# RemoteSensingTools/vSmartMOM.jl

Measured on AMD Instinct MI355X. Metric: spectral-points/s (whole node) for rt_run, O2-A band, higher is better.
Workload: dtype f64

## Files before the change

include/vsmartmom_hip.h:

```cpp
#ifndef VSMARTMOM_HIP_H
#define VSMARTMOM_HIP_H

#include <stddef.h>
#include <stdint.h>

#ifdef __cplusplus
extern "C" {
#endif

typedef enum vsm_status {
  VSM_OK = 0,
  VSM_ERR_INVALID_ARG = 1,
  VSM_ERR_UNSUPPORTED = 2,
  VSM_ERR_HIP = 3,
  VSM_ERR_NO_DEVICE = 4
} vsm_status;

typedef enum vsm_iface {
  VSM_IFACE_00 = 0,
  VSM_IFACE_01 = 1,
  VSM_IFACE_10 = 2,
  VSM_IFACE_11 = 3
} vsm_iface;

// ... 172 lines not shown
int vsm_elemental_lin_mix_f64(const vsm_quad_f64* q, int S, int m, int ndoubl, const double* dtau, const double* varpi,
                              const double* tau_sum, const double* F0, int ncomp, int ncomp_total, const double* Zc_pp,
                              const double* Zc_mp, int zsel, const double* fz, int p_layer, const double* dtau_dot,
                              const double* varpi_dot, const double* tau_sum_dot, const double* zdcoef,
                              const vsm_added_f64* added, const vsm_added_lin_f64* added_lin, void* stream);
int vsm_elemental_lin_mix_f32(const vsm_quad_f32* q, int S, int m, int ndoubl, const float* dtau, const float* varpi,
                              const float* tau_sum, const float* F0, int ncomp, int ncomp_total, const float* Zc_pp,
                              const float* Zc_mp, int zsel, const float* fz, int p_layer, const float* dtau_dot,
                              const float* varpi_dot, const float* tau_sum_dot, const float* zdcoef,
                              const vsm_added_f32* added, const vsm_added_lin_f32* added_lin, void* stream);
size_t vsm_doubling_lin_work_elems(int N, int S, int P);
int vsm_doubling_lin_f64(int N, int n_stokes, int S, int ndoubl, double* expk, const double* dtau_dot_all, double mu0,
                         int n_active, const vsm_added_f64* added, const vsm_added_lin_f64* added_lin, double* work,
                         void* stream);
int vsm_doubling_lin_f32(int N, int n_stokes, int S, int ndoubl, float* expk, const float* dtau_dot_all, float mu0,
                         int n_active, const vsm_added_f32* added, const vsm_added_lin_f32* added_lin, float* work,
                         void* stream);
size_t vsm_interaction_lin_work_elems(int N, int S, int P);
int vsm_interaction_lin_f64(int iface, int N, int S, const vsm_composite_f64* comp, const vsm_composite_lin_f64* comp_lin,
                            const vsm_added_f64* added, const vsm_added_lin_f64* added_lin, double* work, void* stream);
int vsm_interaction_lin_f32(int iface, int N, int S, const vsm_composite_f32* comp, const vsm_composite_lin_f32* comp_lin,
                            const vsm_added_f32* added, const vsm_added_lin_f32* added_lin, float* work, void* stream);
int vsm_interaction_lin_range_f64(int iface, int N, int S, const vsm_composite_f64* comp, const vsm_composite_lin_f64* comp_lin,
                                  const vsm_added_f64* added, const vsm_added_lin_f64* added_lin, int p_lo, int p_hi, double* work,
                                  void* stream);
int vsm_interaction_lin_range_f32(int iface, int N, int S, const vsm_composite_f32* comp, const vsm_composite_lin_f32* comp_lin,
                                  const vsm_added_f32* added, const vsm_added_lin_f32* added_lin, int p_lo, int p_hi, float* work,
                                  void* stream);
int vsm_copy_added_to_composite_lin_f64(int N, int S, const vsm_added_lin_f64* added_lin,
                                        const vsm_composite_lin_f64* comp_lin, void* stream);
int vsm_copy_added_to_composite_lin_f32(int N, int S, const vsm_added_lin_f32* added_lin,
                                        const vsm_composite_lin_f32* comp_lin, void* stream);
int vsm_lambertian_surface_lin_f64(const vsm_quad_f64* q, int S, int m, double albedo, int iparam, const double* tau_sum,
                                   const double* tau_sum_dot, int p_layer, const double* F0, const vsm_added_f64* added,
                                   const vsm_added_lin_f64* added_lin, void* stream);
int vsm_lambertian_surface_lin_f32(const vsm_quad_f32* q, int S, int m, float albedo, int iparam, const float* tau_sum,
                                   const float* tau_sum_dot, int p_layer, const float* F0, const vsm_added_f32* added,
                                   const vsm_added_lin_f32* added_lin, void* stream);
int vsm_postprocess_vza_lin_f64(int N, int n_stokes, int S, int nV, int P, const int* row0_h, const double* w_h,
                                const double* Jdot0_m, const double* Jdot0_p, double* Rdot, double* Tdot, void* stream);
int vsm_postprocess_vza_lin_f32(int N, int n_stokes, int S, int nV, int P, const int* row0_h, const float* w_h,
                                const float* Jdot0_m, const float* Jdot0_p, float* Rdot, float* Tdot, void* stream);

int vsm_lambertian_surface_spectral_f64(const vsm_quad_f64* q, int S, int m, const double* albedo, const double* tau_sum,
                                        const vsm_added_f64* added, void* stream);
int vsm_lambertian_surface_spectral_f32(const vsm_quad_f32* q, int S, int m, const float* albedo, const float* tau_sum,
                                        const vsm_added_f32* added, void* stream);

typedef struct vsm_coxmunk_f64 {
  double wind_speed, n_water_re, n_water_im, whitecap_albedo;
  int include_whitecaps, shadowing;
} vsm_coxmunk_f64;
typedef struct vsm_coxmunk_f32 {
  float wind_speed, n_water_re, n_water_im, whitecap_albedo;
  int include_whitecaps, shadowing;
} vsm_coxmunk_f32;
int vsm_coxmunk_reflectance_f64(const vsm_coxmunk_f64* surf, const vsm_quad_f64* q, int m, int nphi, const double* phi,
                                const double* wphi, double* rho, double* drho_dU, void* stream);
int vsm_coxmunk_reflectance_f32(const vsm_coxmunk_f32* surf, const vsm_quad_f32* q, int m, int nphi, const float* phi,
                                const float* wphi, float* rho, float* drho_dU, void* stream);
int vsm_brdf_surface_f64(const vsm_quad_f64* q, int S, int m, const double* rho, const double* tau_sum,
                         const vsm_added_f64* added, void* stream);
int vsm_brdf_surface_f32(const vsm_quad_f32* q, int S, int m, const float* rho, const float* tau_sum,
                         const vsm_added_f32* added, void* stream);
int vsm_brdf_surface_lin_f64(const vsm_quad_f64* q, int S, int m, const double* rho, const double* drho, int iparam,
                             const double* tau_sum, const double* tau_sum_dot, int p_layer, const double* F0,
                             const vsm_added_f64* added, const vsm_added_lin_f64* added_lin, void* stream);
int vsm_brdf_surface_lin_f32(const vsm_quad_f32* q, int S, int m, const float* rho, const float* drho, int iparam,
                             const float* tau_sum, const float* tau_sum_dot, int p_layer, const float* F0,
                             const vsm_added_f32* added, const vsm_added_lin_f32* added_lin, void* stream);
int vsm_interaction_hdrf_f64(const vsm_quad_f64* q, int S, int m, const vsm_composite_f64* comp,
                             const vsm_added_f64* added_surface, double* hdr_J, double* bhr_uw, double* bhr_dw, void* stream);
int vsm_interaction_hdrf_f32(const vsm_quad_f32* q, int S, int m, const vsm_composite_f32* comp,
                             const vsm_added_f32* added_surface, float* hdr_J, float* bhr_uw, float* bhr_dw, void* stream);
int vsm_postprocess_vza_hdrf_f64(int N, int n_stokes, int S, int nV, const int* row0_h, const double* w_h, const double* hdr_J,
                                 double* hdr, void* stream);
int vsm_postprocess_vza_hdrf_f32(int N, int n_stokes, int S, int nV, const int* row0_h, const float* w_h, const float* hdr_J,
                                 float* hdr, void* stream);
int vsm_coxmunk_ss_correction_f64(const vsm_coxmunk_f64* surf, int n_stokes, int S, int nV, const double* mu_v_h,
                                  const double* dphi_h, double mu0, int m_max, int nphi, const double* phi,
                                  const double* wphi, const double* tau_total, double* coef, double* R_SFI, void* stream);
int vsm_coxmunk_ss_correction_f32(const vsm_coxmunk_f32* surf, int n_stokes, int S, int nV, const float* mu_v_h,
                                  const float* dphi_h, float mu0, int m_max, int nphi, const float* phi, const float* wphi,
                                  const float* tau_total, float* coef, float* R_SFI, void* stream);

int vsm_compute_Z_moments_f64(const vsm_quad_f64* q, int m, int lmax, const double* greek, double* Zpp, double* Zmp,
                              void* stream);
int vsm_compute_Z_moments_f32(const vsm_quad_f32* q, int m, int lmax, const double* greek, float* Zpp, float* Zmp,
                              void* stream);
int vsm_layer_optics_f64(int S, int L, int nAer, const double* tau_rayl, const double* tau_abs, double varpi_cabannes,
                         const double* tau_aer, const double* ssa, const double* ftrunc, const int* mode, double* tau,
                         double* varpi, double* tau_sum, double* fcomp, double* max_tau_varpi, void* stream);
int vsm_layer_optics_f32(int S, int L, int nAer, const double* tau_rayl, const double* tau_abs, double varpi_cabannes,
                         const double* tau_aer, const double* ssa, const double* ftrunc, const int* mode, float* tau,
                         float* varpi, float* tau_sum, float* fcomp, float* max_tau_varpi, void* stream);
int vsm_layer_dtau_f64(int S, int L, const int* ndoubl, const double* tau, double* dtau, void* stream);
int vsm_layer_dtau_f32(int S, int L, const int* ndoubl, const float* tau, float* dtau, void* stream);
int vsm_layer_optics_lin_f64(int S_full, int lo, int S, int L, int nAer, int nGas, int P, const double* tau_rayl,
                             const double* tau_abs, double varpi_cabannes, const double* tau_aer, const double* ssa,
                             const double* ftrunc, const double* tau_abs_dot, const double* tau_aer_dot,
                             const double* ssa_dot, const double* ftrunc_dot, const int* ndoubl, double* dtau_dot_all,
                             double* varpi_dot, double* tau_sum_dot, double* fz, double* zdcoef, void* stream);
int vsm_layer_optics_lin_f32(int S_full, int lo, int S, int L, int nAer, int nGas, int P, const double* tau_rayl,
                             const double* tau_abs, double varpi_cabannes, const double* tau_aer, const double* ssa,
                             const double* ftrunc, const double* tau_abs_dot, const double* tau_aer_dot,
                             const double* ssa_dot, const double* ftrunc_dot, const int* ndoubl, float* dtau_dot_all,
                             float* varpi_dot, float* tau_sum_dot, float* fz, float* zdcoef, void* stream);
int vsm_layer_expk_f64(int S, const double* dtau, double mu0, double* expk, void* stream);
int vsm_layer_expk_f32(int S, const float* dtau, float mu0, float* expk, void* stream);

int vsm_layer_forward_f64(const vsm_quad_f64* q, int S, int m, int ndoubl, const double* dtau, const double* varpi,
                          const double* tau_sum, const double* F0, const double* Zpp, const double* Zmp, long long z_stride,
                          int toa, const vsm_composite_f64* comp, const vsm_added_f64* added_scratch, void* stream);
int vsm_layer_forward_f32(const vsm_quad_f32* q, int S, int m, int ndoubl, const float* dtau, const float* varpi,
                          const float* tau_sum, const float* F0, const float* Zpp, const float* Zmp, long long z_stride,
                          int toa, const vsm_composite_f32* comp, const vsm_added_f32* added_scratch, void* stream);

int vsm_layer_forward_multi_f64(const vsm_quad_f64* q, int S, int nm, const int* m, int ndoubl, const double* dtau,
                                const double* varpi, const double* tau_sum, const double* F0, int ncomp,
                                const double* const* Zpp, const double* const* Zmp, long long z_stride, const double* fcomp,
                                double* z_scratch, int toa, const vsm_composite_f64* comps, const vsm_added_f64* added_scratch,
                                void* stream);
int vsm_layer_forward_multi_f32(const vsm_quad_f32* q, int S, int nm, const int* m, int ndoubl, const float* dtau,
                                const float* varpi, const float* tau_sum, const float* F0, int ncomp, const float* const* Zpp,
                                const float* const* Zmp, long long z_stride, const float* fcomp, float* z_scratch, int toa,
                                const vsm_composite_f32* comps, const vsm_added_f32* added_scratch, void* stream);

int vsm_layer_thermal_fused(int N, int is_f64);
int vsm_layer_forward_thermal_f64(const vsm_quad_f64* q, int S, int ndoubl, const double* dtau, const double* varpi,
                                  const double* thermal_B, int ncomp, const double* Zpp, const double* Zmp, long long z_stride,
                                  const double* fcomp, int toa, const vsm_composite_f64* comp, void* stream);
int vsm_layer_forward_thermal_f32(const vsm_quad_f32* q, int S, int ndoubl, const float* dtau, const float* varpi,
                                  const float* thermal_B, int ncomp, const float* Zpp, const float* Zmp, long long z_stride,
                                  const float* fcomp, int toa, const vsm_composite_f32* comp, void* stream);

int vsm_layer_forward_mix_f64(const vsm_quad_f64* q, int S, int m, int ndoubl, const double* dtau, const double* varpi,
                              const double* tau_sum, const double* F0, int ncomp, const double* Zpp_comp,
                              const double* Zmp_comp, const double* fcomp, double* z_scratch, int toa,
                              const vsm_composite_f64* comp, const vsm_added_f64* added_scratch, void* stream);
int vsm_layer_forward_mix_f32(const vsm_quad_f32* q, int S, int m, int ndoubl, const float* dtau, const float* varpi,
                              const float* tau_sum, const float* F0, int ncomp, const float* Zpp_comp, const float* Zmp_comp,
                              const float* fcomp, float* z_scratch, int toa, const vsm_composite_f32* comp,
                              const vsm_added_f32* added_scratch, void* stream);
int vsm_mix_Z_f64(int N, int S, int ncomp, const double* Zpp_comp, const double* Zmp_comp, const double* fcomp, double* Zpp,
                  double* Zmp, void* stream);
int vsm_mix_Z_f32(int N, int S, int ncomp, const float* Zpp_comp, const float* Zmp_comp, const float* fcomp, float* Zpp,
                  float* Zmp, void* stream);
int vsm_mix_Z_moments_f64(int N, int S, int ncomp, int nm, const double* const* Zpp_comp_h, const double* const* Zmp_comp_h, int single,
                          const double* fcomp, double* Zpp, double* Zmp, void* stream);
int vsm_mix_Z_moments_f32(int N, int S, int ncomp, int nm, const float* const* Zpp_comp_h, const float* const* Zmp_comp_h, int single,
                          const float* fcomp, float* Zpp, float* Zmp, void* stream);

typedef struct vsm_run vsm_run;
enum { VSM_RUN_SOURCES_ONLY = 1 };
int vsm_run_supported(int N, int n_stokes, int coupling);
size_t vsm_run_workspace_bytes(int N, int n_stokes, int S, int nm, const int* coupling_h);
int vsm_run_supported_f32(int N, int n_stokes, int coupling);
size_t vsm_run_workspace_bytes_f32(int N, int n_stokes, int S, int nm, const int* coupling_h);
int vsm_run_create_f64(const vsm_quad_f64* q, int S, int nm, const int* m_h, const int* coupling_h, void* workspace,
                       size_t workspace_bytes, vsm_run** run);
int vsm_run_create_f32(const vsm_quad_f32* q, int S, int nm, const int* m_h, const int* coupling_h, void* workspace,
                       size_t workspace_bytes, vsm_run** run);
int vsm_run_create_ex_f64(const vsm_quad_f64* q, int S, int nm, const int* m_h, const int* coupling_h, void* workspace,
                          size_t workspace_bytes, unsigned flags, vsm_run** run);
int vsm_run_create_ex_f32(const vsm_quad_f32* q, int S, int nm, const int* m_h, const int* coupling_h, void* workspace,
                          size_t workspace_bytes, unsigned flags, vsm_run** run);
int vsm_run_layer_f64(vsm_run* run, int ndoubl, const double* dtau, const double* varpi, const double* tau_sum,
                      const double* F0, int ncomp, const double* const* Zpp, const double* const* Zmp, long long z_stride,
                      const double* fcomp, int toa, const int* layer_coupling_h, void* stream);
int vsm_run_layer_f32(vsm_run* run, int ndoubl, const float* dtau, const float* varpi, const float* tau_sum,
                      const float* F0, int ncomp, const float* const* Zpp, const float* const* Zmp, long long z_stride,
                      const float* fcomp, int toa, const int* layer_coupling_h, void* stream);
int vsm_run_export_f64(vsm_run* run, const vsm_composite_f64* comps, void* stream);
int vsm_run_export_f32(vsm_run* run, const vsm_composite_f32* comps, void* stream);
int vsm_run_import_f64(vsm_run* run, const vsm_composite_f64* comps, void* stream);
int vsm_run_import_f32(vsm_run* run, const vsm_composite_f32* comps, void* stream);
int vsm_run_destroy(vsm_run* run);
int vsm_stokes_coupling_f64(int N, int n_stokes, int nblocks, const double* Zpp, const double* Zmp, int* mask_d, void* stream);
int vsm_stokes_coupling_f32(int N, int n_stokes, int nblocks, const float* Zpp, const float* Zmp, int* mask_d, void* stream);

typedef struct vsm_added_rs_f64 {
  double *ier_mp, *iet_pp, *ier_pm, *iet_mm;
  double *ieJ0_p, *ieJ0_m;
  int K;
  int reserved;
} vsm_added_rs_f64;
typedef struct vsm_added_rs_f32 {
  float *ier_mp, *iet_pp, *ier_pm, *iet_mm;
  float *ieJ0_p, *ieJ0_m;
  int K;
  int reserved;
} vsm_added_rs_f32;
typedef struct vsm_composite_rs_f64 {
  double *ieR_mp, *ieR_pm, *ieT_pp, *ieT_mm;
  double *ieJ0_p, *ieJ0_m;
  int K;
  int reserved;
} vsm_composite_rs_f64;
typedef struct vsm_composite_rs_f32 {
  float *ieR_mp, *ieR_pm, *ieT_pp, *ieT_mm;
  float *ieJ0_p, *ieJ0_m;
  int K;
  int reserved;
} vsm_composite_rs_f32;
typedef struct vsm_rrs_f64 {
  const int* shift;
  const double* varpi_ie;
  const double* fscatt;
  const double* Zpp;
  const double* Zmp;
} vsm_rrs_f64;
typedef struct vsm_rrs_f32 {
  const int* shift;
  const float* varpi_ie;
  const float* fscatt;
  const float* Zpp;
  const float* Zmp;
} vsm_rrs_f32;
int vsm_elemental_inelastic_rrs_f64(const vsm_quad_f64* q, int S, int m, int ndoubl, const double* dtau,
                                    const double* tau_sum, const double* F0, const vsm_rrs_f64* rs,
                                    const vsm_added_rs_f64* added_rs, void* stream);
int vsm_elemental_inelastic_rrs_f32(const vsm_quad_f32* q, int S, int m, int ndoubl, const float* dtau,
                                    const float* tau_sum, const float* F0, const vsm_rrs_f32* rs,
                                    const vsm_added_rs_f32* added_rs, void* stream);
size_t vsm_doubling_inelastic_work_elems(int N, int S, int K);
int vsm_doubling_inelastic_rrs_f64(int N, int n_stokes, int S, int ndoubl, double* expk, const int* shift,
                                   const vsm_added_f64* added, const vsm_added_rs_f64* added_rs, double* work, void* stream);
int vsm_doubling_inelastic_rrs_f32(int N, int n_stokes, int S, int ndoubl, float* expk, const int* shift,
                                   const vsm_added_f32* added, const vsm_added_rs_f32* added_rs, float* work, void* stream);
size_t vsm_interaction_inelastic_work_elems(int N, int S, int K);
int vsm_interaction_inelastic_rrs_f64(int iface, int N, int S, const int* shift, const vsm_composite_f64* comp,
                                      const vsm_composite_rs_f64* comp_rs, const vsm_added_f64* added,
                                      const vsm_added_rs_f64* added_rs, double* work, void* stream);
int vsm_interaction_inelastic_rrs_f32(int iface, int N, int S, const int* shift, const vsm_composite_f32* comp,
                                      const vsm_composite_rs_f32* comp_rs, const vsm_added_f32* added,
                                      const vsm_added_rs_f32* added_rs, float* work, void* stream);
int vsm_copy_added_to_composite_ie_f64(int N, int S, const vsm_added_rs_f64* added_rs, const vsm_composite_rs_f64* comp_rs,
                                       void* stream);
int vsm_copy_added_to_composite_ie_f32(int N, int S, const vsm_added_rs_f32* added_rs, const vsm_composite_rs_f32* comp_rs,
                                       void* stream);
int vsm_postprocess_vza_ie_f64(int N, int n_stokes, int S, int K, int nV, const int* row0_h, const double* w_h,
                               const double* ieJ0_m, const double* ieJ0_p, double* ieR, double* ieT, void* stream);
int vsm_postprocess_vza_ie_f32(int N, int n_stokes, int S, int K, int nV, const int* row0_h, const float* w_h,
                               const float* ieJ0_m, const float* ieJ0_p, float* ieR, float* ieT, void* stream);

size_t vsm_level_radiance_work_elems(int N, int S);
int vsm_level_radiance_f64(int N, int n_stokes, int S, int nV, const int* row0_h, const double* w_h, const double* top_R_pm,
                           const double* top_J0_p, const double* bot_R_mp, long long bot_stride, const double* bot_J0_m,
                           double* uw, double* dw, double* dw_full, double* uw_full, double* work, void* stream);
int vsm_level_radiance_f32(int N, int n_stokes, int S, int nV, const int* row0_h, const float* w_h, const float* top_R_pm,
                           const float* top_J0_p, const float* bot_R_mp, long long bot_stride, const float* bot_J0_m,
                           float* uw, float* dw, float* dw_full, float* uw_full, float* work, void* stream);
int vsm_level_radiance_oplevel_f64(int N, int n_stokes, int S, int nV, const int* row0_h, const double* w_h,
                                   const double* top_R_pm, const double* top_J0_p, const double* bot_R_mp, long long bot_stride,
                                   const double* bot_J0_m, double* uw, double* dw, double* dw_full, double* uw_full,
                                   double* work, void* stream);
int vsm_level_radiance_oplevel_f32(int N, int n_stokes, int S, int nV, const int* row0_h, const float* w_h,
                                   const float* top_R_pm, const float* top_J0_p, const float* bot_R_mp, long long bot_stride,
                                   const float* bot_J0_m, float* uw, float* dw, float* dw_full, float* uw_full, float* work,
                                   void* stream);

int vsm_test_lds_mm_f64(int N, int S, const double* A, const double* B, double* C, void* stream);
int vsm_test_lds_mm_f32(int N, int S, const float* A, const float* B, float* C, void* stream);
int vsm_test_lds_inv_f64(int N, int S, const double* A, double* X, int mode, int* path_out, void* stream);
int vsm_test_lds_inv_f32(int N, int S, const float* A, float* X, int mode, int* path_out, void* stream);

int vsm_test_poison_lds(void* stream);

#ifdef __cplusplus
}
#endif
#endif
```

vsmartmom.jl_amd/_lib.py:

```python
from __future__ import annotations

import ctypes as C
import os

_HERE = os.path.dirname(os.path.abspath(__file__))
LIB_PATH = os.environ.get("VSM_LIB_PATH") or os.path.join(_HERE, "lib", "libvsmartmom_hip.so")


class VSMError(RuntimeError):
    pass


class vsm_quad_f64(C.Structure):
    _fields_ = [("mu", C.c_void_p), ("wt", C.c_void_p), ("N", C.c_int), ("n_stokes", C.c_int),
                ("i_mu0", C.c_int), ("mu0", C.c_double)]


class vsm_quad_f32(C.Structure):
    _fields_ = [("mu", C.c_void_p), ("wt", C.c_void_p), ("N", C.c_int), ("n_stokes", C.c_int),
                ("i_mu0", C.c_int), ("mu0", C.c_float)]


class vsm_added(C.Structure):
    _fields_ = [("r_mp", C.c_void_p), ("t_pp", C.c_void_p), ("r_pm", C.c_void_p), ("t_mm", C.c_void_p),
                ("j0_p", C.c_void_p), ("j0_m", C.c_void_p), ("mat_stride", C.c_longlong),
                ("d_symmetric", C.c_int), ("reserved", C.c_int)]


class vsm_composite(C.Structure):
    _fields_ = [("R_mp", C.c_void_p), ("R_pm", C.c_void_p), ("T_pp", C.c_void_p), ("T_mm", C.c_void_p),
                ("J0_p", C.c_void_p), ("J0_m", C.c_void_p)]


class vsm_added_lin(C.Structure):
    _fields_ = [("ap_r_mp", C.c_void_p), ("ap_t_pp", C.c_void_p), ("ap_r_pm", C.c_void_p), ("ap_t_mm", C.c_void_p),
                ("ap_J0_p", C.c_void_p), ("ap_J0_m", C.c_void_p), ("P", C.c_int), ("reserved", C.c_int),
                ("mat_stride", C.c_longlong)]


class vsm_composite_lin(C.Structure):
    _fields_ = [("R_mp", C.c_void_p), ("R_pm", C.c_void_p), ("T_pp", C.c_void_p), ("T_mm", C.c_void_p),
                ("J0_p", C.c_void_p), ("J0_m", C.c_void_p), ("P", C.c_int), ("reserved", C.c_int)]


class vsm_added_rs(C.Structure):
    _fields_ = [("ier_mp", C.c_void_p), ("iet_pp", C.c_void_p), ("ier_pm", C.c_void_p), ("iet_mm", C.c_void_p),
                ("ieJ0_p", C.c_void_p), ("ieJ0_m", C.c_void_p), ("K", C.c_int), ("reserved", C.c_int)]


class vsm_composite_rs(C.Structure):
    _fields_ = [("ieR_mp", C.c_void_p), ("ieR_pm", C.c_void_p), ("ieT_pp", C.c_void_p), ("ieT_mm", C.c_void_p),
                ("ieJ0_p", C.c_void_p), ("ieJ0_m", C.c_void_p), ("K", C.c_int), ("reserved", C.c_int)]


class vsm_coxmunk_f64(C.Structure):
    _fields_ = [("wind_speed", C.c_double), ("n_water_re", C.c_double), ("n_water_im", C.c_double),
                ("whitecap_albedo", C.c_double), ("include_whitecaps", C.c_int), ("shadowing", C.c_int)]


class vsm_coxmunk_f32(C.Structure):
    _fields_ = [("wind_speed", C.c_float), ("n_water_re", C.c_float), ("n_water_im", C.c_float),
                ("whitecap_albedo", C.c_float), ("include_whitecaps", C.c_int), ("shadowing", C.c_int)]


class vsm_rrs(C.Structure):
    _fields_ = [("shift", C.c_void_p), ("varpi_ie", C.c_void_p), ("fscatt", C.c_void_p), ("Zpp", C.c_void_p),
                ("Zmp", C.c_void_p)]


_P, _I, _LL, _SZ = C.c_void_p, C.c_int, C.c_longlong, C.c_size_t

_SIGS = {
    "vsm_version": (_I, []),
    "vsm_last_error": (C.c_char_p, []),
    "vsm_build_id": (C.c_char_p, []),
    "vsm_device_count": (_I, [C.POINTER(_I)]),
    "vsm_device_name": (_I, [_I, C.c_char_p, _SZ]),
    "vsm_sync": (_I, [_P]),
    "vsm_release_scratch": (_I, []),
    "vsm_device_status": (_I, [C.POINTER(_I), _I, _P]),
    "vsm_fused_max_n": (_I, [_I]),
    "vsm_layer_thermal_fused": (_I, [_I, _I]),
    "vsm_doubling_work_elems": (_SZ, [_I, _I]),
    "vsm_interaction_work_elems": (_SZ, [_I, _I]),
    "vsm_batched_mul_{T}": (_I, [_I, _I, _I, _I, _P, _LL, _P, _LL, _P, _P]),
    "vsm_batch_inv_{T}": (_I, [_I, _I, _P, _P, _P, _P]),
    "vsm_batch_solve_{T}": (_I, [_I, _I, _I, _P, _P, _P, _P, _P, _P]),
    "vsm_elemental_doubling_{T}": (_I, [_P, _I, _I, _I, _P, _P, _P, _P, _P, _P, _LL, _P, _P]),
    "vsm_layer_forward_{T}": (_I, [_P, _I, _I, _I, _P, _P, _P, _P, _P, _P, _LL, _I, _P, _P, _P]),
    "vsm_layer_forward_multi_{T}": (_I, [_P, _I, _I, _P, _I, _P, _P, _P, _P, _I, _P, _P, _LL, _P, _P, _I, _P, _P, _P]),
    "vsm_layer_forward_thermal_{T}": (_I, [_P, _I, _I, _P, _P, _P, _I, _P, _P, _LL, _P, _I, _P, _P]),
    "vsm_layer_forward_mix_{T}": (_I, [_P, _I, _I, _I, _P, _P, _P, _P, _I, _P, _P, _P, _P, _I, _P, _P, _P]),
    "vsm_mix_Z_{T}": (_I, [_I, _I, _I, _P, _P, _P, _P, _P, _P]),
    "vsm_mix_Z_moments_{T}": (_I, [_I, _I, _I, _I, _P, _P, _I, _P, _P, _P, _P]),
    "vsm_elemental_{T}": (_I, [_P, _I, _I, _I, _P, _P, _P, _P, _P, _P, _LL, _P, _P]),
    "vsm_doubling_{T}": (_I, [_I, _I, _I, _I, _P, _P, _P, _P]),
    "vsm_noscat_layer_{T}": (_I, [_P, _I, _P, _P, _P]),
    "vsm_thermal_source_{T}": (_I, [_P, _I, _P, _P, _P, _P, _P]),
    "vsm_copy_added_to_composite_{T}": (_I, [_I, _I, _P, _P, _P]),
    "vsm_interaction_{T}": (_I, [_I, _I, _I, _P, _P, _P, _P]),
    "vsm_interaction_oplevel_{T}": (_I, [_I, _I, _I, _P, _P, _P, _P]),
    "vsm_lambertian_surface_{T}": (_I, [_P, _I, _I, "{R}", _P, _P, _P]),
    "vsm_postprocess_vza_{T}": (_I, [_I, _I, _I, _I, _P, _P, _P, _P, _P, _P, _P]),
    "vsm_compute_Z_moments_{T}": (_I, [_P, _I, _I, _P, _P, _P, _P]),
    "vsm_layer_optics_{T}": (_I, [_I, _I, _I, _P, _P, C.c_double, _P, _P, _P, _P, _P, _P, _P, _P, _P, _P]),
    "vsm_layer_dtau_{T}": (_I, [_I, _I, _P, _P, _P, _P]),
    "vsm_layer_optics_lin_{T}": (_I, [_I, _I, _I, _I, _I, _I, _I, _P, _P, C.c_double, _P, _P, _P, _P, _P, _P, _P, _P, _P, _P, _P,
                                      _P, _P, _P]),
    "vsm_layer_expk_{T}": (_I, [_I, _P, "{R}", _P, _P]),
    "vsm_coxmunk_reflectance_{T}": (_I, [_P, _P, _I, _I, _P, _P, _P, _P, _P]),
    "vsm_lambertian_surface_spectral_{T}": (_I, [_P, _I, _I, _P, _P, _P, _P]),
    "vsm_brdf_surface_{T}": (_I, [_P, _I, _I, _P, _P, _P, _P]),
    "vsm_brdf_surface_lin_{T}": (_I, [_P, _I, _I, _P, _P, _I, _P, _P, _I, _P, _P, _P, _P]),
    "vsm_interaction_hdrf_{T}": (_I, [_P, _I, _I, _P, _P, _P, _P, _P, _P]),
    "vsm_postprocess_vza_hdrf_{T}": (_I, [_I, _I, _I, _I, _P, _P, _P, _P, _P]),
    "vsm_coxmunk_ss_correction_{T}": (_I, [_P, _I, _I, _I, _P, _P, "{R}", _I, _I, _P, _P, _P, _P, _P, _P]),
    "vsm_doubling_lin_work_elems": (_SZ, [_I, _I, _I]),
    "vsm_interaction_lin_work_elems": (_SZ, [_I, _I, _I]),
    "vsm_elemental_lin_{T}": (_I, [_P, _I, _I, _I, _P, _P, _P, _P, _P, _P, _LL, _I, _P, _P, _P, _P, _P, _LL, _LL, _P, _P, _P]),
    "vsm_elemental_lin_fold_{T}": (_I, [_P, _I, _I, _I, _I, _P, _P, _P, _P, _P, _P, _LL, _I, _P, _P, _P, _P, _P, _P]),
    "vsm_elemental_lin_mix_{T}": (_I, [_P, _I, _I, _I, _P, _P, _P, _P, _I, _I, _P, _P, _I, _P, _I, _P, _P, _P, _P, _P, _P, _P]),
    "vsm_doubling_lin_{T}": (_I, [_I, _I, _I, _I, _P, _P, "{R}", _I, _P, _P, _P, _P]),
    "vsm_interaction_lin_{T}": (_I, [_I, _I, _I, _P, _P, _P, _P, _P, _P]),
    "vsm_interaction_lin_range_{T}": (_I, [_I, _I, _I, _P, _P, _P, _P, _I, _I, _P, _P]),
    "vsm_copy_added_to_composite_lin_{T}": (_I, [_I, _I, _P, _P, _P]),
    "vsm_lambertian_surface_lin_{T}": (_I, [_P, _I, _I, "{R}", _I, _P, _P, _I, _P, _P, _P, _P]),
    "vsm_postprocess_vza_lin_{T}": (_I, [_I, _I, _I, _I, _I, _P, _P, _P, _P, _P, _P, _P]),
    "vsm_doubling_inelastic_work_elems": (_SZ, [_I, _I, _I]),
    "vsm_interaction_inelastic_work_elems": (_SZ, [_I, _I, _I]),
    "vsm_elemental_inelastic_rrs_{T}": (_I, [_P, _I, _I, _I, _P, _P, _P, _P, _P, _P]),
    "vsm_doubling_inelastic_rrs_{T}": (_I, [_I, _I, _I, _I, _P, _P, _P, _P, _P, _P]),
    "vsm_interaction_inelastic_rrs_{T}": (_I, [_I, _I, _I, _P, _P, _P, _P, _P, _P, _P]),
    "vsm_copy_added_to_composite_ie_{T}": (_I, [_I, _I, _P, _P, _P]),
    "vsm_postprocess_vza_ie_{T}": (_I, [_I, _I, _I, _I, _I, _P, _P, _P, _P, _P, _P, _P]),
    "vsm_run_supported": (_I, [_I, _I, _I]),
    "vsm_run_workspace_bytes": (_SZ, [_I, _I, _I, _I, _P]),
    "vsm_run_supported_f32": (_I, [_I, _I, _I]),
    "vsm_run_workspace_bytes_f32": (_SZ, [_I, _I, _I, _I, _P]),
    "vsm_run_create_{T}": (_I, [_P, _I, _I, _P, _P, _P, _SZ, _P]),
    "vsm_run_create_ex_{T}": (_I, [_P, _I, _I, _P, _P, _P, _SZ, C.c_uint, _P]),
    "vsm_run_layer_{T}": (_I, [_P, _I, _P, _P, _P, _P, _I, _P, _P, _LL, _P, _I, _P, _P]),
    "vsm_run_export_{T}": (_I, [_P, _P, _P]),
    "vsm_run_import_{T}": (_I, [_P, _P, _P]),
    "vsm_run_destroy": (_I, [_P]),
    "vsm_stokes_coupling_{T}": (_I, [_I, _I, _I, _P, _P, _P, _P]),
    "vsm_level_radiance_work_elems": (_SZ, [_I, _I]),
    "vsm_level_radiance_{T}": (_I, [_I, _I, _I, _I, _P, _P, _P, _P, _P, _LL, _P, _P, _P, _P, _P, _P, _P]),
    "vsm_level_radiance_oplevel_{T}": (_I, [_I, _I, _I, _I, _P, _P, _P, _P, _P, _LL, _P, _P, _P, _P, _P, _P, _P]),
    "vsm_test_lds_mm_{T}": (_I, [_I, _I, _P, _P, _P, _P]),
    "vsm_test_lds_inv_{T}": (_I, [_I, _I, _P, _P, _I, _P, _P]),
    "vsm_test_poison_lds": (_I, [_P]),
}


def exported_symbols():
    out = []
    for name in _SIGS:
        if "{T}" in name:
            out += [name.format(T="f64"), name.format(T="f32")]
        else:
            out.append(name)
    return out


_lib = None


def lib():
    global _lib
    if _lib is not None:
        return _lib
    if not os.path.exists(LIB_PATH):
        raise VSMError("libvsmartmom_hip.so not found at %s -- run `python -c 'import __graft_entry__ as g; g.build()'` "
                       "(there is no CPU fallback)" % LIB_PATH)
    L = C.CDLL(LIB_PATH)
    for name, (res, args) in _SIGS.items():
        for T, R in (("f64", C.c_double), ("f32", C.c_float)):
            n = name.format(T=T)
            try:
                fn = getattr(L, n)
            except AttributeError:
                if os.environ.get("VSM_LIB_PATH"):
                    if "{T}" not in name:
                        break
                    continue
                raise
            fn.restype = res
            fn.argtypes = [R if a == "{R}" else a for a in args]
            if "{T}" not in name:
                break
    _lib = L
    return L


def build_info() -> dict:
    import json
    info = {"source_hash": lib().vsm_build_id().decode() if hasattr(lib(), "vsm_build_id") else None}
    try:
        with open(os.path.join(os.path.dirname(LIB_PATH), "BUILD_INFO.json")) as f:
            side = json.load(f)
        if side.get("source_hash") == info["source_hash"]:
            info.update(side)
    except (OSError, ValueError):
        pass
    return info


def poison(t):
    if os.environ.get("VSM_POISON_WORK"):
        t.fill_(float("nan"))
    return t


def check(rc):
    if rc != 0:
        raise VSMError("libvsmartmom_hip: status %d: %s" % (rc, lib().vsm_last_error().decode()))


last_device_status = [0, 0, 0, 0]


def check_device_status(what="rt_run"):
    global last_device_status
    flags = (C.c_int * 4)()
    check(lib().vsm_device_status(flags, 1, None))
    last_device_status = list(flags)
    if flags[0] & 1:
        raise VSMError("%s: singular matrix in an in-kernel inverse ((I - R r) or (I - r r) has an exactly zero pivot)" % what)
    if flags[0] & 2:
        raise VSMError("%s: NaN / Inf operand in an in-kernel inverse" % what)
    if flags[0] & 4:
        raise VSMError("%s: a phase matrix handed to vsm_run_layer has a non-zero element outside the declared Stokes coupling "
                       "(VSM_DEVSTAT_MASK): the native run dropped that coupling" % what)


def suffix(dtype) -> str:
    import torch
    if dtype == torch.float64:
        return "f64"
    if dtype == torch.float32:
        return "f32"
    raise VSMError("unsupported float type %r (Float64 / Float32 only)" % (dtype,))


def call(name, dtype, *args):
    fn = getattr(lib(), "%s_%s" % (name, suffix(dtype)))
    check(fn(*args))
```

vsmartmom.jl_amd/core_rt.py:

```python
from __future__ import annotations

import ctypes as C
import dataclasses
import math
import os
from dataclasses import dataclass
from typing import List, Optional

import numpy as np
import torch

from . import _lib
from . import host_model as H
from .architectures import GPU, CPU, architecture, array_type, devi, synchronize_if_gpu, to_host

IFACE = {"00": 0, "01": 1, "10": 2, "11": 3}
MOMENT_BATCH = 4
MOMENT_BATCH_MAX = 24
MOMENT_BATCHING = True
THERMAL_FUSION = True
NATIVE_RUN = True
NATIVE_SOURCES_ONLY = True
NATIVE_DROPIN = True
REFERENCE_ORDER = False


def _require_gpu(arch):
    if not isinstance(arch, GPU):
        raise _lib.VSMError("vsmartmom.jl_amd provides the MI355X path only; architecture %r has no compute path here "
                            "(no CPU fallback by design)" % (arch,))
    if not torch.cuda.is_available():
        raise _lib.VSMError("no MI355X visible to HIP (torch.cuda.is_available() is False)")
    if arch.device_index != torch.cuda.current_device():
        raise _lib.VSMError("architecture GPU(%d) is not the current HIP device (%d): one process per GPU -- call "
                            "torch.cuda.set_device(%d) first" % (arch.device_index, torch.cuda.current_device(),
                                                                 arch.device_index))


def _torch_dtype(FT):
    return torch.float64 if np.dtype(FT) == np.float64 else torch.float32


def _stream_ptr():
    return C.c_void_p(torch.cuda.current_stream().cuda_stream)


def _ptr(t: Optional[torch.Tensor]):
    return C.c_void_p(0 if t is None else t.data_ptr())


def to_device_matrix(A: np.ndarray, arch, FT) -> torch.Tensor:
    A = np.asarray(A, dtype=FT)
    if A.ndim == 2:
        A = A[None]
    return array_type(arch)(np.ascontiguousarray(A.transpose(0, 2, 1)))


def from_device_matrix(t: torch.Tensor) -> np.ndarray:
    return to_host(t).transpose(0, 2, 1).copy()


def batched_mul(A: torch.Tensor, B: torch.Tensor) -> torch.Tensor:
    _require_gpu(architecture(A))
    vec = B.dim() == 2
    S, K, M = A.shape
    Nc = 1 if vec else B.shape[1]
    kb = B.shape[1] if vec else B.shape[2]
    if kb != K or B.shape[0] not in (S, 1):
        raise _lib.VSMError("batched_mul: dimension mismatch %s x %s" % (tuple(A.shape), tuple(B.shape)))
    A, B = A.contiguous(), B.contiguous()
    Cout = torch.empty((S, M) if vec else (S, Nc, M), dtype=A.dtype, device=A.device)
    sb = 0 if B.shape[0] == 1 and S > 1 else K * Nc
    _lib.call("vsm_batched_mul", A.dtype, M, Nc, K, S, _ptr(A), M * K, _ptr(B), sb, _ptr(Cout), _stream_ptr())
    return Cout


def batch_inv_(X: torch.Tensor, A: torch.Tensor, info: Optional[torch.Tensor] = None):
    _require_gpu(architecture(A))
    S, N, N2 = A.shape
    if N != N2 or X.shape != A.shape:
        raise _lib.VSMError("batch_inv!: square batches of equal shape required")
    _lib.call("vsm_batch_inv", A.dtype, N, S, _ptr(A), _ptr(X), _ptr(info), _stream_ptr())
    return X


def batch_solve_(X: torch.Tensor, A: torch.Tensor, B: torch.Tensor, info: Optional[torch.Tensor] = None):
    _require_gpu(architecture(A))
    S, N, N2 = A.shape
    nrhs = 1 if B.dim() == 2 else B.shape[1]
    if N != N2 or B.shape[0] != S or B.shape[-1] != N or X.shape != B.shape:
        raise _lib.VSMError("batch_solve!: A [N,N,S] and B, X [N,Nrhs,S] required")
    work = _lib.poison(torch.empty_like(A))
    _lib.call("vsm_batch_solve", A.dtype, N, nrhs, S, _ptr(A.contiguous()), _ptr(B.contiguous()), _ptr(X), _ptr(work), _ptr(info),
              _stream_ptr())
    return X


def batched_pointer_cache(A):
    return None


@dataclass
class DeviceQuad:
    host: H.QuadPoints
    mu: torch.Tensor
    wt: torch.Tensor
    n_stokes: int
    dtype: torch.dtype

    def cstruct(self):
        cls = _lib.vsm_quad_f64 if self.dtype == torch.float64 else _lib.vsm_quad_f32
        return cls(self.mu.data_ptr(), self.wt.data_ptr(), int(self.mu.numel()), self.n_stokes, self.host.imu0,
                   self.host.mu0)


def device_quad(qp: H.QuadPoints, pol: H.PolarizationType, arch, FT) -> DeviceQuad:
    conv = array_type(arch)
    return DeviceQuad(qp, conv(qp.qp_muN.astype(FT)), conv(qp.wt_muN.astype(FT)), pol.n, _torch_dtype(FT))


class AddedLayer:

    def __init__(self, FT, arch, N, nSpec, shared=False, d_symmetric=0):
        dev, dt = devi(arch), _torch_dtype(FT)
        sm = 1 if shared else nSpec
        z = lambda: torch.zeros((sm, N, N), dtype=dt, device=dev)
        self.r_mp, self.t_pp = z(), z()
        self.d_symmetric = int(d_symmetric)
        self.r_pm, self.t_mm = (None, None) if self.d_symmetric else (z(), z())
        self.j0_p = torch.zeros((nSpec, N), dtype=dt, device=dev)
        self.j0_m = torch.zeros((nSpec, N), dtype=dt, device=dev)
        self.N, self.nSpec, self.shared, self.dtype = N, nSpec, shared, dt

    def cstruct(self):
        return _lib.vsm_added(self.r_mp.data_ptr(), self.t_pp.data_ptr(),
                              0 if self.r_pm is None else self.r_pm.data_ptr(),
                              0 if self.t_mm is None else self.t_mm.data_ptr(),
                              self.j0_p.data_ptr(), self.j0_m.data_ptr(), 0 if self.shared else self.N * self.N,
                              self.d_symmetric, 0)


def _composite_field(name):
    def fget(self):
        return self.materialize()._arr[name]

    def fset(self, value):
        self.materialize()._arr[name] = value
    return property(fget, fset)


class CompositeLayer:

    def __init__(self, FT, arch, N, nSpec):
        dev, dt = devi(arch), _torch_dtype(FT)
        z = lambda: torch.zeros((nSpec, N, N), dtype=dt, device=dev)
        self._native = None
        self._sources_only = False
        self._native_ws = None
        self._arr = dict(R_mp=z(), R_pm=z(), T_pp=z(), T_mm=z(), J0_p=torch.zeros((nSpec, N), dtype=dt, device=dev),
                         J0_m=torch.zeros((nSpec, N), dtype=dt, device=dev))
        self.N, self.nSpec, self.dtype = N, nSpec, dt

    R_mp, R_pm, T_pp = _composite_field("R_mp"), _composite_field("R_pm"), _composite_field("T_pp")
    T_mm, J0_p, J0_m = _composite_field("T_mm"), _composite_field("J0_p"), _composite_field("J0_m")

    def materialize(self):
        slot = self._native
        if slot is None:
            return self
        self._native = None
        try:
            cc = (_lib.vsm_composite * 1)(self._cstruct_raw())
            _lib.call("vsm_run_export", self.dtype, slot.run, cc, _stream_ptr())
        finally:
            _lib.lib().vsm_run_destroy(slot.run)
# ... 578 lines not shown
                key = (type(model.surface).__name__, dataclasses.astuple(model.surface), m)
                cache = self.__dict__.setdefault("_rho_cache", {})
                if key not in cache:
                    if len(cache) > 4 * (model.m_max + 1):
                        cache.clear()
                    cache[key] = reflectance(model.surface, self.dq, m, self.arch, FT)[0]
                rho = cache[key]
            self.moments.append(dict(m=m, layers=layers, iface_surface=tags[-1], rho=rho, tau_sum_surface=self.tau_sum[L, lo:hi]))
        all11 = all(t == "11" for t in tags)
        fused_ok = self.N <= _lib.lib().vsm_fused_max_n(8 if np.dtype(FT) == np.float64 else 4)
        dsym = self.pol.n if (all11 and fused_ok and not self.full_added_layer) else 0
        if self.added is None or self.added.d_symmetric != dsym:
            self.added = make_added_layer(FT, self.arch, (self.N, self.N), self.S, d_symmetric=dsym)

    def _prepare_host(self):
        model, FT, L, S_full = self.model, self.FT, self.Nz, self.S_full
        conv = array_type(self.arch)
        nds = tags = maxima = None
        for m in range(model.m_max + 1):
            Zc_pp, Zc_mp, lods = H.constructLayerOpticsComponents(model, m)
            self.Zc[m][0].copy_(to_device_matrix(Zc_pp, self.arch, FT))
            self.Zc[m][1].copy_(to_device_matrix(Zc_mp, self.arch, FT))
            if m > 0:
                continue
            tags, tau_sum_all = H.extractEffectiveProps(lods, FT)
            nds, maxima = [], []
            zcomp = []
            for iz, lo in enumerate(lods):
                tau_full = np.atleast_1d(lo.tau).astype(FT)
                varpi_full = np.broadcast_to(np.asarray(lo.varpi, dtype=FT), tau_full.shape)
                tw = float(np.max(tau_full * varpi_full))
                scatter = tw > 2 * np.finfo(FT).eps
                dtau_full, nd = (H.get_dtau_ndoubl(tau_full, varpi_full, self.qp, FT, model.numerics) if scatter else (tau_full, 0))
                nds.append(nd)
                maxima.append(tw)
                self.tau[iz].copy_(conv(tau_full))
                self.varpi[iz].copy_(conv(np.ascontiguousarray(varpi_full)))
                self.dtau[iz].copy_(conv(np.ascontiguousarray(dtau_full)))
                self.tau_sum[iz].copy_(conv(tau_sum_all[:, iz].astype(FT)))
                if lo.coef.ndim == 1:
                    zcomp.append((False, int(np.argmax(lo.coef))))
                else:
                    zcomp.append((True, 0))
                    self.fcomp[iz].copy_(conv(np.ascontiguousarray(lo.coef.astype(FT))))
            self.tau_sum[L].copy_(conv(tau_sum_all[:, -1].astype(FT)))
            self.zcomp = zcomp
        self._compute_coupling()
        self._assemble(nds, tags, maxima)

    def _compute_coupling(self):
        C_ = int(self.Zc[0][0].shape[0])
        if not self.host_optics and getattr(self, "coupling_comp", None) is not None:
            return
        if getattr(self, "_coupling_d", None) is None:
            self._coupling_d = torch.zeros((len(self.Zc), C_), dtype=torch.int32, device=self.dev)
        for m, (Zpp, Zmp) in enumerate(self.Zc):
            _lib.call("vsm_stokes_coupling", self.dt, self.N, self.pol.n, C_, _ptr(Zpp), _ptr(Zmp),
                      C.c_void_p(self._coupling_d[m].data_ptr()), _stream_ptr())
        self.coupling_comp = self._coupling_d.cpu().numpy().astype(np.int64)
        self.coupling = [int(np.bitwise_or.reduce(row)) for row in self.coupling_comp]

    def _layer_coupling(self, m, iz):
        mixed, k = self.zcomp[iz]
        row = self.coupling_comp[m]
        return int(np.bitwise_or.reduce(row)) if mixed else int(row[k])

    def run(self, trace: Optional[list] = None, streams: Optional[list] = None):
        model, pol, FT = self.model, self.pol, self.FT
        self.R_SFI.zero_()
        self.T_SFI.zero_()
        self.hdr.zero_()
        if self.S == 0:
            return self.R_SFI, self.T_SFI
        self.added.j0_p.zero_()
        eps2 = 2 * np.finfo(FT).eps
        has_noscat = any(ly["props"].max_tau_varpi <= eps2 for ly in self.moments[0]["layers"])
        sequential = trace is not None or not MOMENT_BATCHING or has_noscat or REFERENCE_ORDER
        want = max(MOMENT_BATCH, min(MOMENT_BATCH_MAX, 4096 // max(self.S, 1)))
        nb = 1 if sequential else min(want, len(self.moments))
        while len(self._composites) < nb:
            self._composites.append(make_composite_layer(FT, self.arch, (self.N, self.N), self.S))
        native = self._native_moments() if trace is None and not has_noscat and not REFERENCE_ORDER else set()
        walk_src = streams is None and trace is None and not has_noscat
        for c in self._composites:
            c._sources_only = walk_src and REFERENCE_ORDER
        for g0 in range(0, len(self.moments), nb):
            group = self.moments[g0:g0 + nb]
            comps = self._composites[:len(group)]
            nat = [k for k in range(len(group)) if (g0 + k) in native]
            if nat:
                self._run_layers_native([group[k] for k in nat], [comps[k] for k in nat], sources_only=streams is None)
            rest = [k for k in range(len(group)) if (g0 + k) not in native]
            group_l, comps_l = [group[k] for k in rest], [comps[k] for k in rest]
            for iz in range(self.Nz if rest else 0):
                ly0 = group_l[0]["layers"][iz]
                if len(group_l) > 1 and ly0["props"].max_tau_varpi > eps2 and (iz == 0 or ly0["iface"] == "11"):
                    layer_forward_multi_(ly0["tau_sum"], ly0["dtau"], self.F0, [mom["layers"][iz]["props"] for mom in group_l],
                                         [mom["m"] for mom in group_l], ly0["nd"], self.dq, iz == 0, comps_l, self.added)
                    continue
                for mom, comp in zip(group_l, comps_l):
                    ly = mom["layers"][iz]
                    rt_kernel_(pol, self.added, comp, ly["props"], ly["iface"], ly["tau_sum"], mom["m"], self.dq,
                               self.arch, iz + 1, self.F0, FT, model.numerics, dtau=ly["dtau"], ndoubl=ly["nd"], trace=trace,
                               work=self.work, keep_added=has_noscat)
            for mom, comp in zip(group, comps):
                m = mom["m"]
                weight = FT(0.5 / math.pi) if m == 0 else FT(1.0 / math.pi)
                create_surface_layer_(model.surface, self.added_surface, m, self.dq, mom["tau_sum_surface"], rho=mom["rho"])
                interaction_(mom["iface_surface"], comp, self.added_surface, work=self.work)
                if self.compute_hdrf:
                    interaction_hdrf_(pol, comp, self.added_surface, m, self.dq, model.vza, model.vaz, self.qp, float(weight),
                                      self.hdr_J, self.hdr, self.bhr_uw, self.bhr_dw)
                postprocessing_vza_(pol, comp, model.vza, model.vaz, self.qp, m, float(weight), self.R_SFI, self.T_SFI)
                thermal_pass = self.thermal_B is not None and (m == 0 or (m == 1 and self._thermal_carry))
                if thermal_pass:
                    self._thermal_slot(mom, float(weight))
                if streams is not None:
                    Jm, Jp = comp.J0_m.clone(), comp.J0_p.clone()
                    if thermal_pass:
                        Jm += self._th_comp.J0_m
                        Jp += self._th_comp.J0_p
                    streams.append(dict(m=m, weight=float(weight), R_mp=comp.R_mp.clone(), T_pp=comp.T_pp.clone(), J0_m=Jm, J0_p=Jp))
        for c in self._composites:
            c._sources_only = False
        if isinstance(model.surface, H.CoxMunkSurface) and self.ss_correction:
            apply_ss_correction_(self.R_SFI, model.surface, pol, model.vza, model.vaz, self.qp.mu0,
                                 self.moments[-1]["tau_sum_surface"], model.m_max, self.arch, FT)
        return self.R_SFI, self.T_SFI

    def _native_moments(self):
        if not NATIVE_RUN or getattr(self, "coupling", None) is None or not self.moments:
            return set()
        eps2 = 2 * np.finfo(self.FT).eps
        for iz, ly in enumerate(self.moments[0]["layers"]):
            p = ly["props"]
            if p.max_tau_varpi <= eps2 or (iz > 0 and ly["iface"] != "11") or (p.fcomp is not None and p.fcomp.shape[1] > 4):
                return set()
        return {i for i, mom in enumerate(self.moments) if run_supported(self.dt, self.N, self.pol.n, int(self.coupling[mom["m"]]))}

    def _run_layers_native(self, group, comps, sources_only: bool = True, export_at=None):
        L = _lib.lib()
        nm, N, S, ns = len(group), self.N, self.S, self.pol.n
        marr = (C.c_int * nm)(*[int(mom["m"]) for mom in group])
        carr = (C.c_int * nm)(*[int(self.coupling[mom["m"]]) for mom in group])
        nbytes = run_workspace_bytes(self.dt, N, ns, S, nm, carr)
        ws = getattr(self, "_native_ws", None)
        if ws is None or ws.numel() * 8 < nbytes:
            ws = self._native_ws = _lib.poison(torch.empty(max(nbytes // 8, 2), dtype=torch.float64, device=self.dev))
        q = self.dq.cstruct()
        run = C.c_void_p()
        flags = 1 if (sources_only and NATIVE_SOURCES_ONLY) else 0
        _lib.call("vsm_run_create_ex", self.dt, C.byref(q), S, nm, marr, carr, _ptr(ws), nbytes, flags, C.byref(run))
        try:
            for iz in range(self.Nz):
                ly0 = group[0]["layers"][iz]
                props = [mom["layers"][iz]["props"] for mom in group]
                p0 = props[0]
                zpp = (C.c_void_p * nm)(*[p.Zpp.data_ptr() for p in props])
                zmp = (C.c_void_p * nm)(*[p.Zmp.data_ptr() for p in props])
                ncomp = 0 if p0.fcomp is None else int(p0.fcomp.shape[1])
                lc = (C.c_int * nm)(*[self._layer_coupling(mom["m"], iz) for mom in group])
                run_layer_native_(run, nm, int(ly0["nd"]), ly0["dtau"], p0.varpi, ly0["tau_sum"], self.F0, ncomp, zpp, zmp,
                                  0 if ncomp else p0.z_stride, p0.fcomp, iz == 0, lc, self.dt)
                if export_at and (iz + 1) in export_at:
                    cc = (type(comps[0].cstruct()) * nm)(*[c.cstruct() for c in comps])
                    _lib.call("vsm_run_export", self.dt, run, cc, _stream_ptr())
                    export_at[iz + 1](comps)
            cc = (type(comps[0].cstruct()) * nm)(*[c.cstruct() for c in comps])
            _lib.call("vsm_run_export", self.dt, run, cc, _stream_ptr())
        finally:
            L.vsm_run_destroy(run)

    def _thermal_slot(self, mom, weight):
        model, pol, FT = self.model, self.pol, self.FT
        N, S = self.N, self.S
        m = mom["m"]
        if getattr(self, "_th_added", None) is None:
            self._th_added = make_added_layer(FT, self.arch, (N, N), S, d_symmetric=0)
            self._th_surf = make_added_layer(FT, self.arch, (N, N), S, shared=not self.spectral_surface)
            self._th_comp = make_composite_layer(FT, self.arch, (N, N), S)
            self._th_F0 = torch.zeros_like(self.F0)
            self._th_ones = torch.ones(max(S, 1), dtype=self.dt, device=self.dev)
        added, comp = self._th_added, self._th_comp
        q = self.dq.cstruct()
        eps2 = 2 * np.finfo(FT).eps
        scat = [ly["props"].max_tau_varpi > eps2 for ly in mom["layers"]]
        keep_state = not self.thermal_reset_noscat
        if m == 0:
            added.j0_p.zero_()
            added.j0_m.zero_()
            self._thermal_carry = keep_state and any(scat) and not scat[0] and model.m_max >= 1
        fused = (THERMAL_FUSION and m == 0 and (all(scat) or not keep_state)
                 and _lib.lib().vsm_layer_thermal_fused(N, 1 if FT == np.float64 else 0) != 0)
        for iz, ly in enumerate(mom["layers"]):
            props = ly["props"]
            scatter = scat[iz]
            if (fused and scatter and (iz == 0 or ly["iface"] == "11") and iz < self.thermal_B.shape[0]
                    and (props.fcomp is None or props.fcomp.shape[1] <= 4)):
                c = comp.cstruct()
                ncomp = 0 if props.fcomp is None else int(props.fcomp.shape[1])
                _lib.call("vsm_layer_forward_thermal", self.dt, C.byref(q), S, ly["nd"], _ptr(ly["dtau"]), _ptr(props.varpi),
                          _ptr(self.thermal_B[iz]), ncomp, _ptr(props.Zpp), _ptr(props.Zmp),
                          0 if ncomp else props.z_stride, _ptr(props.fcomp), 1 if iz == 0 else 0, C.byref(c), _stream_ptr())
                continue
            if scatter:
                elemental_(pol, ly["tau_sum"], ly["dtau"], self._th_F0, props.materialize(), m, ly["nd"], self.dq, added)
                if m == 0 and iz < self.thermal_B.shape[0]:
                    a = added.cstruct()
                    _lib.call("vsm_thermal_source", self.dt, C.byref(q), S, _ptr(ly["dtau"]), _ptr(props.varpi),
                              _ptr(self.thermal_B[iz]), C.byref(a), _stream_ptr())
                self._th_ones.fill_(1.0)
                doubling_(pol, self._th_ones, ly["nd"], added)
            elif keep_state:
                jm = added.j0_m.clone()
                zero_added_noscat_(added, props.tau, self.dq)
                added.j0_m.copy_(jm)
            else:
                zero_added_noscat_(added, props.tau, self.dq)
                added.j0_p.zero_()
                added.j0_m.zero_()
            if iz == 0:
                copy_added_to_composite_(comp, added)
            else:
                interaction_(ly["iface"], comp, added, oplevel=True, work=self.work)
        create_surface_layer_(model.surface, self._th_surf, m, self.dq, mom["tau_sum_surface"], rho=mom["rho"])
        self._th_surf.j0_p.zero_()
        self._th_surf.j0_m.zero_()
        interaction_(mom["iface_surface"], comp, self._th_surf, oplevel=True, work=self.work)
        postprocessing_vza_(pol, comp, model.vza, model.vaz, self.qp, m, weight, self.R_SFI, self.T_SFI)

    def run_graph(self):
        if getattr(self, "_graph", None) is None:
            if self.added.d_symmetric == 0 or any(ly["props"].fcomp is not None for ly in self.moments[0]["layers"]):
                raise _lib.VSMError("run_graph(): only scenes that run entirely in the fused layer kernels (every layer "
                                    "scattering, N within the on-chip limit, one scatterer per layer) can be captured")
            gs = torch.cuda.Stream()
            gs.wait_stream(torch.cuda.current_stream())
            with torch.cuda.stream(gs):
                self.run()
            torch.cuda.synchronize()
            g = torch.cuda.CUDAGraph()
            with torch.cuda.graph(g, stream=gs):
                self.run()
            self._graph, self._graph_stream = g, gs
        self._graph.replay()
        return self.R_SFI, self.T_SFI

    def results_host(self):
        return to_host(self.R_SFI).transpose(2, 1, 0).copy(), to_host(self.T_SFI).transpose(2, 1, 0).copy()

    def results_host_full(self):
        R, T = self.results_host()
        return (R, T, np.zeros_like(R), np.zeros_like(T), to_host(self.hdr).transpose(2, 1, 0).copy(),
                to_host(self.bhr_uw)[:, 0].copy(), to_host(self.bhr_dw)[:, 0].copy())

    def flops_per_point(self) -> float:
        N = float(self.N)
        tot = 0.0
        for mom in self.moments:
            for iz, ly in enumerate(mom["layers"]):
                tot += ly["nd"] * (12 * N ** 3 + 8 * N ** 2)
                if iz > 0:
                    tot += 24 * N ** 3 + 8 * N ** 2
            tot += 24 * N ** 3 + 8 * N ** 2
        return tot


def prepare_scene(model: H.RTModel, spec_slice: Optional[slice] = None) -> Scene:
    return Scene(model, spec_slice)


@dataclass
class StreamRTResult:
    qp_mu: np.ndarray
    i_mu0: int
    mu0: float
    pol_n: int
    weight: List[float]
    R_mp_per_m: List[np.ndarray]
    T_pp_per_m: List[np.ndarray]
    J_m_per_m: List[np.ndarray]
    J_p_per_m: List[np.ndarray]
    tau_total: np.ndarray
    tau_rayl: np.ndarray
    tau_abs: np.ndarray


def rt_run_streams(model: H.RTModel) -> StreamRTResult:
    scene = prepare_scene(model)
    scene.compute_hdrf = False
    st: list = []
    scene.run(streams=st)
    synchronize_if_gpu()
    st.sort(key=lambda d: d["m"])
    mat = lambda t: from_device_matrix(t).transpose(1, 2, 0).copy()
    vec = lambda t: to_host(t).T[:, None, :].copy()
    qp = model.quad_points
    FT = model.float_type
    return StreamRTResult(np.asarray(qp.qp_mu, dtype=FT).copy(), int(qp.imu0) + 1, float(qp.mu0), model.polarization_type.n,
                          [d["weight"] for d in st], [mat(d["R_mp"]) for d in st], [mat(d["T_pp"]) for d in st],
                          [vec(d["J0_m"]) for d in st], [vec(d["J0_p"]) for d in st],
                          (np.asarray(model.tau_rayl) + np.asarray(model.tau_abs)).astype(FT), np.asarray(model.tau_rayl, dtype=FT),
                          np.asarray(model.tau_abs, dtype=FT))


def rt_run(model: H.RTModel, trace: Optional[list] = None, full_output: bool = False):
# ... 7 lines not shown
```

vsmartmom.jl_amd/csrc/vsm_native.hip:

```cpp
#include <stdlib.h>

#include <vector>

#include "vsm_native_dev.h"
#include "vsm_native_run.h"

#ifndef VSM_NATIVE_PARK_RT
#define VSM_NATIVE_PARK_RT 3
#endif

namespace vsm {

struct nlayer_comps {
  double* c[NSUB_MAX];
};

namespace {

template <int RT, int KS>
__device__ __forceinline__ void ned_body(nsmem<RT, (4 * KS + 2 > 16 * RT)>& sm, npos<RT>& p, int n, int gsz, unsigned uvmask, int ndoubl,
                                         const double* __restrict__ img, nstrip<RT>& r_s, nstrip<RT>& t_s, int* status) {
  using G = ngeo<RT>;
  constexpr unsigned dP = 0, dQ = G::AF * 8;
  double* jp = sm.vec[0];
  double* jm = sm.vec[1];
  double* rsg = sm.vec[3];
  const int tid = threadIdx.x;
  constexpr int c1 = 4 * KS, c2 = 4 * KS + 1;
  constexpr bool RID = c2 < G::NP;
  static_assert(RID || KS == 4 * RT, "no spare columns for the source vectors");
  const bool own_wave = RID && p.wave == (c1 >> 4);
  const bool laneA = own_wave && (p.col == c1), laneB = own_wave && (p.col == c2), laneAB = laneA || laneB;
  ncopy_image<RT>(sm.P, img, p);
  ncopy_image<RT>(sm.Q, img + G::AF, p);
  if (tid < G::NP) {
    jp[tid] = img[2 * G::AF + tid];
    jm[tid] = img[2 * G::AF + G::NP + tid];
    const bool uv = (uvmask >> (tid % gsz)) & 1u;
    sm.usg[tid] = uv ? -1.0 : 1.0;
    rsg[tid] = (ndoubl >= 1 && uv) ? -1.0 : 1.0;
  }
  const double expk0 = img[2 * G::AF + 2 * G::NP];
  __builtin_amdgcn_s_waitcnt(0x0F70);
  __syncthreads();
  nload(r_s, dP, p);
  nload(t_s, dQ, p);
  double expk = expk0;
  int slot = 0;
  const ninv_ctx cx{dP, sm.P, sm.gjs, status};
  for (int it = 0; it < ndoubl; ++it) {
    nstrip<RT> W, tt;
    const double fW = laneA ? expk : (laneB ? 1.0 : 0.0), fR = laneB ? expk : 1.0;
    if constexpr (!RID) {
      nmv_rows<RT, KS>(dP, jp, 1.0, sm.mv[0], p);
      nmv_rows<RT, KS>(dP, jm, expk, sm.mv[1], p);
    }
    {
      nstrip<RT> Gs;
      {
        nstrip<RT> E;
        nmm2<RT, KS, true, true>(E, W, dP, r_s, t_s, p);
        if (own_wave) {
#pragma unroll
          for (int ta = 0; ta < RT; ++ta)
#pragma unroll
            for (int r = 0; r < 4; ++r) {
              W.v[ta][r] = fma(r_s.v[ta][r], fW, W.v[ta][r]);
              r_s.v[ta][r] *= fR;
            }
        }
        const double nrm = nnorm(E, n, sm, slot, p);
        if constexpr (!RID) {
          if (tid < G::NP) {
            sm.vec[4][tid] = jm[tid] * expk + sm.mv[0][tid];
            sm.vec[5][tid] = jp[tid] + sm.mv[1][tid];
          }
        }
        ninvert<RT, KS>(ninv_order(nrm, status), E, Gs, n, cx, p);
      }
      nmm<RT, KS, true>(tt, dQ, Gs, p);
    }
    nload(t_s, dQ, p);
    __syncthreads();
    nstore(dP, tt, p);
    __syncthreads();
    if constexpr (!RID) {
      nmv_rows<RT, KS>(dP, sm.vec[4], 1.0, sm.mv[0], p);
      nmv_rows<RT, KS>(dP, sm.vec[5], 1.0, sm.mv[1], p);
    }
    {
      nstrip<RT> tn;
      nmm2<RT, KS, false, true>(r_s, tn, dP, W, t_s, p);
      t_s = tn;
    }
    const double expk_step = expk;
    expk = expk * expk;
    if (own_wave) {
      const double ft = laneB ? expk : 1.0;
#pragma unroll
      for (int ta = 0; ta < RT; ++ta)
#pragma unroll
        for (int r = 0; r < 4; ++r) {
          const double u = ndpp_swap1(r_s.v[ta][r]) * ft;
          t_s.v[ta][r] = laneAB ? u : t_s.v[ta][r];
        }
    }
    if (it + 1 < ndoubl || !RID) __syncthreads();
    if constexpr (!RID) {
      if (tid < G::NP) {
        jm[tid] += sm.mv[0][tid];
        jp[tid] = jp[tid] * expk_step + sm.mv[1][tid];
      }
    }
    if (it + 1 < ndoubl) {
      nstore(dP, r_s, p);
      nstore(dQ, t_s, p);
      __syncthreads();
    }
  }
  if (ndoubl > 0 && own_wave) {
#pragma unroll
    for (int ta = 0; ta < RT; ++ta)
#pragma unroll
      for (int r = 0; r < 4; ++r) {
        const int row = p.row(ta, r);
        double* dpv = laneA ? jp : sm.vec[7];
        double* dmv = laneA ? jm : sm.vec[7];
        dpv[row] = t_s.v[ta][r];
        dmv[row] = r_s.v[ta][r];
        t_s.v[ta][r] = laneAB ? 0.0 : t_s.v[ta][r];
        r_s.v[ta][r] = laneAB ? 0.0 : r_s.v[ta][r];
      }
  }
  __syncthreads();
  if (ndoubl >= 1) {
#pragma unroll
    for (int ta = 0; ta < RT; ++ta)
#pragma unroll
      for (int r = 0; r < 4; ++r) r_s.v[ta][r] *= rsg[p.row(ta, r)];
    if (tid < G::NP) jm[tid] *= rsg[tid];
  }
  __syncthreads();
}

template <int RT, int KS>
__device__ __forceinline__ void nia_body_native(nsmem<RT, (4 * KS + 2 > 16 * RT)>& sm, npos<RT>& p, int n, double* __restrict__ comp, nstrip<RT>& r_s,
                                         nstrip<RT>& t_s, int* status) {
  using G = ngeo<RT>;
  constexpr unsigned dP = 0, dQ = G::AF * 8;
  double* vjp = sm.vec[0];
  double* vjm = sm.vec[1];
  double* vJp = sm.vec[2];
  double* vJm = sm.vec[3];
  double* vs = sm.vec[4];
  double* vz = sm.vec[5];
  const int tid = threadIdx.x;
  double* R_mp = comp + NC_RMP * G::AF;
  double* R_pm = comp + NC_RPM * G::AF;
  double* T_pp = comp + NC_TPP * G::AF;
  double* T_mm = comp + NC_TMM * G::AF;
  double* J0_p = comp + 4 * G::AF;
  double* J0_m = J0_p + G::NP;
  constexpr int c1 = 4 * KS, c2 = 4 * KS + 1;
  constexpr bool RID = c2 < G::NP;
  constexpr bool PARK = VSM_NATIVE_PARK_RT > 0 && (RT == VSM_NATIVE_PARK_RT || RT >= 5);
  const bool own_wave = RID && p.wave == (c1 >> 4);
  const bool laneA = own_wave && (p.col == c1), laneB = own_wave && (p.col == c2);
  int slot = 0;
  const ndpar<RT> dp(sm.usg, p);
  const ninv_ctx cx{dP, sm.P, sm.gjs, status};
  if (tid < G::NP) {
    vJp[tid] = J0_p[tid];
    vJm[tid] = J0_m[tid];
  }
  nstrip<RT> Z, Gs;
  {
    nstrip<RT> A1, A2;
    nld_native(A1, R_pm, p);
    nld_native(A2, T_mm, p);
    nstore(dP, A1, p);
    nstore(dQ, A2, p);
  }
  if (own_wave) {
#pragma unroll
    for (int ta = 0; ta < RT; ++ta)
#pragma unroll
      for (int r = 0; r < 4; ++r) r_s.v[ta][r] = laneB ? vjm[p.row(ta, r)] : r_s.v[ta][r];
  }
  ndsym(t_s, t_s, dp);
  __syncthreads();
  if constexpr (!RID) {
    nmv_rows<RT, KS>(dP, vjm, 1.0, sm.mv[0], p);
    nmv_rows<RT, KS>(dQ, vjm, 1.0, sm.mv[1], p);
  }
  {
    nstrip<RT> E;
    nmm2<RT, KS, true, true>(E, Z, dP, r_s, t_s, p);
    if (own_wave) {
      double* zd = laneB ? vz : sm.vec[7];
#pragma unroll
      for (int ta = 0; ta < RT; ++ta)
#pragma unroll
        for (int r = 0; r < 4; ++r) {
          const int row = p.row(ta, r);
          zd[row] = vJp[row] + E.v[ta][r];
        }
    }
    if constexpr (PARK) nst_native(R_pm, Z, p);
    const double nrm = nnorm(E, n, sm, slot, p);
    if constexpr (!RID) {
      if (tid < G::NP) {
        vz[tid] = vJp[tid] + sm.mv[0][tid];
        vs[tid] = sm.mv[1][tid];
      }
    }
    ninvert<RT, KS>(ninv_order(nrm, status), E, Gs, n, cx, p);
  }
  nstrip<RT> V;
  {
    nstrip<RT> S;
    nmm2<RT, KS, true, true>(S, V, dQ, r_s, t_s, p);
    if (own_wave) {
      double* sd = laneB ? vs : sm.vec[7];
#pragma unroll
      for (int ta = 0; ta < RT; ++ta)
#pragma unroll
        for (int r = 0; r < 4; ++r) sd[p.row(ta, r)] = S.v[ta][r];
    }
    ndsym(r_s, r_s, dp);
    ndsym(t_s, t_s, dp);
    __syncthreads();
    nstore(dQ, S, p);
    nstore(dP, t_s, p);
  }
  __syncthreads();
  {
    nstrip<RT> X, Y;
    nmm<RT, KS, true>(X, dP, Gs, p);
    nmm<RT, KS, true>(Y, dQ, Gs, p);
    __syncthreads();
    nstore(dP, X, p);
    nstore(dQ, Y, p);
  }
  __builtin_amdgcn_sched_barrier(0);
  nstrip<RT> Tpp, Rmp;
  nld_native(Tpp, T_pp, p);
  if constexpr (PARK) nld_native(Z, R_pm, p); else nld_native(Rmp, R_mp, p);
  __syncthreads();
  if constexpr (!RID) {
    nmv_rows<RT, KS>(dP, vz, 1.0, sm.mv[0], p);
    nmv_rows<RT, KS>(dQ, vz, 1.0, sm.mv[1], p);
  }
  if (own_wave) {
#pragma unroll
    for (int ta = 0; ta < RT; ++ta)
#pragma unroll
      for (int r = 0; r < 4; ++r) {
        Tpp.v[ta][r] = laneA ? vz[p.row(ta, r)] : Tpp.v[ta][r];
        if constexpr (!PARK) Rmp.v[ta][r] = laneA ? 0.0 : Rmp.v[ta][r];
      }
  }
  {
    nstrip<RT> acc;
    nmm2<RT, KS, false, true>(r_s, acc, dP, Z, Tpp, p);
    nst_native(R_pm, r_s, p);
    nst_native(T_pp, acc, p);
    if (laneA) {
#pragma unroll
      for (int ta = 0; ta < RT; ++ta)
#pragma unroll
        for (int r = 0; r < 4; ++r) {
          const int row = p.row(ta, r);
          J0_p[row] = vjp[row] + acc.v[ta][r];
        }
    }
  }
  if constexpr (PARK) {
    __builtin_amdgcn_sched_barrier(0);
    nld_native(Rmp, R_mp, p);
    if (own_wave) {
#pragma unroll
      for (int ta = 0; ta < RT; ++ta)
#pragma unroll
        for (int r = 0; r < 4; ++r) Rmp.v[ta][r] = laneA ? 0.0 : Rmp.v[ta][r];
    }
  }
  nmm2<RT, KS>(Rmp, V, dQ, Tpp, Z, p);
  nst_native(R_mp, Rmp, p);
  nst_native(T_mm, V, p);
  if (laneA) {
#pragma unroll
    for (int ta = 0; ta < RT; ++ta)
#pragma unroll
      for (int r = 0; r < 4; ++r) {
        const int row = p.row(ta, r);
        J0_m[row] = vJm[row] + vs[row] + Rmp.v[ta][r];
      }
  }
  if constexpr (!RID) {
    __syncthreads();
    if (tid < G::NP) {
      J0_p[tid] = vjp[tid] + sm.mv[0][tid];
      J0_m[tid] = vJm[tid] + vs[tid] + sm.mv[1][tid];
    }
  }
}

template <int RT, int KS>
__device__ __forceinline__ void nia_body_src(nsmem<RT, (4 * KS + 2 > 16 * RT)>& sm, npos<RT>& p, int n, double* __restrict__ comp,
                                             nstrip<RT>& r_s, nstrip<RT>& t_s, int* status) {
  using G = ngeo<RT>;
  constexpr unsigned dP = 0, dQ = G::AF * 8;
  double* vjp = sm.vec[0];
  double* vjm = sm.vec[1];
  double* vJp = sm.vec[2];
  double* vJm = sm.vec[3];
  double* vu = sm.vec[4];
  double* vtJ = sm.vec[5];
  double* vg = sm.vec[6];
  const int tid = threadIdx.x;
  double* R_pm = comp + NC_RPM * G::AF;
  double* T_mm = comp + NC_TMM * G::AF;
  double* J0_p = comp + 4 * G::AF;
  double* J0_m = J0_p + G::NP;
  constexpr int c1 = 4 * KS, c2 = 4 * KS + 1;
  constexpr bool RID = c2 < G::NP;
  const bool own_wave = RID && p.wave == (c1 >> 4);
  const bool laneA = own_wave && (p.col == c1);
  constexpr bool PARK = VSM_NATIVE_PARK_RT > 0 && (RT == VSM_NATIVE_PARK_RT || RT >= 5);
  int slot = 0;
  const ndpar<RT> dp(sm.usg, p);
  const ninv_ctx cx{dP, sm.P, sm.gjs, status};
  if (tid < G::NP) {
    vJp[tid] = J0_p[tid];
    vJm[tid] = J0_m[tid];
  }
  nstrip<RT> B;
  nld_native(B, R_pm, p);
  nstore(dP, r_s, p);
  nstore(dQ, t_s, p);
  __syncthreads();
  {
    const bool cin = p.col < n;
#pragma unroll
    for (int ta = 0; ta < RT; ++ta)
#pragma unroll
      for (int r = 0; r < 4; ++r) B.v[ta][r] = cin ? B.v[ta][r] : (laneA ? vJp[p.row(ta, r)] : 0.0);
  }
  if constexpr (!RID) {
    nmv_rows<RT, KS>(dP, vJp, 1.0, sm.mv[0], p);
    nmv_rows<RT, KS>(dQ, vJp, 1.0, sm.mv[1], p);
  }
  nstrip<RT> E, Bs;
  double nrm;
  {
    nstrip<RT> Pm;
    nmm2a<RT, KS, true, true>(E, dP, Pm, dQ, B, p);
    ndsym(Bs, t_s, dp);
    ndsym(r_s, r_s, dp);
    if (own_wave) {
#pragma unroll
      for (int ta = 0; ta < RT; ++ta)
#pragma unroll
        for (int r = 0; r < 4; ++r) {
          const int row = p.row(ta, r);
          Bs.v[ta][r] = laneA ? E.v[ta][r] + vjm[row] : Bs.v[ta][r];
          r_s.v[ta][r] = laneA ? Pm.v[ta][r] + vjp[row] : r_s.v[ta][r];
        }
    }
    if constexpr (PARK) nst_native(R_pm, r_s, p);
    nrm = nnorm(E, n, sm, slot, p);
    nstore(dQ, Pm, p);
  }
  if constexpr (!RID) {
    if (tid < G::NP) {
      vu[tid] = sm.mv[0][tid] + vjm[tid];
      vtJ[tid] = sm.mv[1][tid] + vjp[tid];
    }
  }
  nstrip<RT> W;
  {
    nstrip<RT> Gs;
    const int K = ninv_order(nrm, status);
    if (K == 7) ninvert7<RT, KS>(E, Gs, n, cx, p);
    else ninvert<RT, KS>(K, E, Gs, n, cx, p);
    __syncthreads();
    nstore(dP, Gs, p);
  }
  __syncthreads();
  if constexpr (!RID) nmv_rows<RT, KS>(dP, vu, 1.0, vg, p);
  {
    nstrip<RT> Tm;
    nld_native(Tm, T_mm, p);
    if constexpr (PARK) nld_native(r_s, R_pm, p);
    nmm<RT, KS, true>(W, dP, Bs, p);
    __syncthreads();
    nstore(dP, Tm, p);
  }
  __syncthreads();
  if constexpr (!RID) {
    nmv_rows<RT, KS>(dP, vg, 1.0, sm.mv[0], p);
    nmv_rows<RT, KS>(dQ, vg, 1.0, sm.mv[1], p);
  }
  {
    nstrip<RT> Tn;
    nmm2a<RT, KS, true, false>(Tn, dP, r_s, dQ, W, p);
    nst_native(R_pm, r_s, p);
    nst_native(T_mm, Tn, p);
    if (laneA) {
#pragma unroll
      for (int ta = 0; ta < RT; ++ta)
#pragma unroll
        for (int r = 0; r < 4; ++r) {
          const int row = p.row(ta, r);
          J0_p[row] = r_s.v[ta][r];
          J0_m[row] = vJm[row] + Tn.v[ta][r];
        }
    }
  }
  if constexpr (!RID) {
    __syncthreads();
    if (tid < G::NP) {
      J0_m[tid] = vJm[tid] + sm.mv[0][tid];
      J0_p[tid] = vtJ[tid] + sm.mv[1][tid];
    }
  }
}

template <int RT>
struct nio_ref {
  int N;
  double* m[4];
  double* J[2];
  const double* a[4];
  double jpre[2];
  bool al16;
  static constexpr bool REF = true;
  static __device__ __forceinline__ void swap16(double& a, double& b) {
    const unsigned long long ua = __double_as_longlong(a), ub = __double_as_longlong(b);
    const auto lo = __builtin_amdgcn_permlane16_swap((unsigned)ua, (unsigned)ub, false, false);
    const auto hi = __builtin_amdgcn_permlane16_swap((unsigned)(ua >> 32), (unsigned)(ub >> 32), false, false);
    a = __longlong_as_double(((unsigned long long)hi[0] << 32) | lo[0]);
    b = __longlong_as_double(((unsigned long long)hi[1] << 32) | lo[1]);
  }
  typedef double npair16_t __attribute__((ext_vector_type(2)));
  typedef double npair8_t __attribute__((ext_vector_type(2), aligned(8)));
  template <typename PT>
  __device__ __forceinline__ void ldg_even(nstrip<RT>& x, const double* __restrict__ gc, bool cok, int rb) const {
#pragma unroll
    for (int ta = 0; ta < RT; ++ta)
#pragma unroll
      for (int h = 0; h < 2; ++h) {
        const int row = 16 * ta + 8 * h + rb;
        const PT v = *reinterpret_cast<const PT*>(gc + min(row, N - 2));
        const bool ok = cok && row < N;
        double a = ok ? v.x : 0.0, b = ok ? v.y : 0.0;
        swap16(a, b);
        x.v[ta][2 * h] = a;
        x.v[ta][2 * h + 1] = b;
      }
  }
  __device__ __forceinline__ void ldg(nstrip<RT>& x, const double* __restrict__ g, const npos<RT>& p) const {
    const bool cok = p.col < N;
    const int rb = 4 * (p.kq & 1) + 2 * (p.kq >> 1);
    const double* gc = g + (long long)N * min(p.col, N - 1);
    if (al16) {
      ldg_even<npair16_t>(x, gc, cok, rb);
      return;
    }
    if ((N & 1) == 0) {
      ldg_even<npair8_t>(x, gc, cok, rb);
      return;
    }
#pragma unroll
    for (int ta = 0; ta < RT; ++ta)
#pragma unroll
      for (int h = 0; h < 2; ++h) {
        const int row = 16 * ta + 8 * h + rb;
        double a = 0.0, b = 0.0;
        if (cok && row + 1 < N) {
          const npair8_t v = *reinterpret_cast<const npair8_t*>(gc + row);
          a = v.x;
          b = v.y;
        } else if (cok && row < N) {
          a = gc[row];
        }
        swap16(a, b);
        x.v[ta][2 * h] = a;
        x.v[ta][2 * h + 1] = b;
      }
  }
  __device__ __forceinline__ void ld(nstrip<RT>& x, int which, const npos<RT>& p) const { ldg(x, m[which], p); }
  __device__ __forceinline__ void ld_added(nstrip<RT>& x, int which, const npos<RT>& p) const { ldg(x, a[which], p); }
  template <typename PT>
  __device__ __forceinline__ void st_even(double* gc, const nstrip<RT>& x, bool cok, int rb) const {
#pragma unroll
    for (int ta = 0; ta < RT; ++ta)
#pragma unroll
      for (int h = 0; h < 2; ++h) {
        double a = x.v[ta][2 * h], b = x.v[ta][2 * h + 1];
        swap16(a, b);
        const int row = 16 * ta + 8 * h + rb;
        if (cok && row < N) {
          PT v;
          v.x = a;
          v.y = b;
          *reinterpret_cast<PT*>(gc + row) = v;
        }
      }
  }
  __device__ __forceinline__ void st(int which, const nstrip<RT>& x, const npos<RT>& p) const {
    const int rb = 4 * (p.kq & 1) + 2 * (p.kq >> 1);
    double* gc = m[which] + (long long)N * min(p.col, N - 1);
    const bool cok = p.col < N;
    if (al16) {
      st_even<npair16_t>(gc, x, cok, rb);
      return;
    }
    if ((N & 1) == 0) {
      st_even<npair8_t>(gc, x, cok, rb);
      return;
    }
#pragma unroll
    for (int ta = 0; ta < RT; ++ta)
#pragma unroll
      for (int h = 0; h < 2; ++h) {
        double a = x.v[ta][2 * h], b = x.v[ta][2 * h + 1];
        swap16(a, b);
        const int row = 16 * ta + 8 * h + rb;
        if (cok && row + 1 < N) {
          npair8_t v;
          v.x = a;
          v.y = b;
          *reinterpret_cast<npair8_t*>(gc + row) = v;
        } else if (cok && row < N) {
          gc[row] = a;
        }
      }
  }
  __device__ __forceinline__ double ldJ(int pm, int) const { return jpre[pm]; }
  __device__ __forceinline__ void stJ(int pm, int i, double v) const {
    if (i < N) J[pm][i] = v;
  }
  __device__ __forceinline__ void dma_raw(const double* __restrict__ g, double* L, const npos<RT>& p) const {
    if (al16) {
      const int chunks = (N * N) >> 1;
      for (int c0 = 64 * p.wave; c0 < chunks; c0 += ngeo<RT>::NT) {
        if (c0 + p.lane < chunks)
          __builtin_amdgcn_global_load_lds((const __attribute__((address_space(1))) void*)(g + 2 * (c0 + p.lane)),
                                           (__attribute__((address_space(3))) void*)(L + 2 * c0), 16, 0, 0);
      }
    } else {
      const int chunks = 2 * N * N;
      const float* g4 = reinterpret_cast<const float*>(g);
      float* L4 = reinterpret_cast<float*>(L);
      for (int c0 = 64 * p.wave; c0 < chunks; c0 += ngeo<RT>::NT) {
        if (c0 + p.lane < chunks)
          __builtin_amdgcn_global_load_lds((const __attribute__((address_space(1))) void*)(g4 + c0 + p.lane),
                                           (__attribute__((address_space(3))) void*)(L4 + c0), 4, 0, 0);
// ... 143 lines not shown
    __syncthreads();
    if constexpr (!RID) {
      if (tid < G::NP) vs[tid] = sm.mv[1][tid];
    }
    nstore(dQ, S, p);
    nstore(dP, t_s, p);
  }
  __syncthreads();
  io.prefetch(NC_RMP, sm.gjs);
  VSM_IA_STAMP(5);
  nstrip<RT> Tpp;
  {
    nstrip<RT> X, Y;
    nmm<RT, KS, true>(X, dP, Gs, p);
    nmm<RT, KS, true>(Y, dQ, Gs, p);
    VSM_IA_STAMP(6);
    __syncthreads();
    io.dma_raw(io.m[NC_TPP], sm.P, p);
    nstore(dQ, Y, p);
    __builtin_amdgcn_s_waitcnt(0x0F70);
    __syncthreads();
    io.ld_raw(Tpp, sm.P, p);
    __syncthreads();
    nstore(dP, X, p);
  }
  __builtin_amdgcn_sched_barrier(0);
  nstrip<RT> Rmp;
  __syncthreads();
  VSM_IA_STAMP(7);
  if constexpr (!RID) {
    nmv_rows<RT, KS>(dP, vz, 1.0, sm.mv[0], p);
    nmv_rows<RT, KS>(dQ, vz, 1.0, sm.mv[1], p);
  }
  if (own_wave) {
#pragma unroll
    for (int ta = 0; ta < RT; ++ta)
#pragma unroll
      for (int r = 0; r < 4; ++r) {
        Tpp.v[ta][r] = laneA ? vz[p.row(ta, r)] : Tpp.v[ta][r];
      }
  }
  {
    nstrip<RT> acc;
    nmm2<RT, KS, false, true>(r_s, acc, dP, Z, Tpp, p);
    VSM_IA_STAMP(8);
    io.ld(Rmp, NC_RMP, p);
    io.st(NC_RPM, r_s, p);
    io.st(NC_TPP, acc, p);
    if (laneA) {
#pragma unroll
      for (int ta = 0; ta < RT; ++ta)
#pragma unroll
        for (int r = 0; r < 4; ++r) {
          const int row = p.row(ta, r);
          io.stJ(0, row, vjp[row] + acc.v[ta][r]);
        }
    }
  }
  VSM_IA_STAMP(9);
  {
    nstrip<RT> YT;
    nmm2<RT, KS, true, false>(YT, V, dQ, Tpp, Z, p);
    VSM_IA_STAMP(10);
#pragma unroll
    for (int ta = 0; ta < RT; ++ta)
#pragma unroll
      for (int r = 0; r < 4; ++r) Rmp.v[ta][r] += YT.v[ta][r];
  }
  io.st(NC_RMP, Rmp, p);
  io.st(NC_TMM, V, p);
  if (laneA) {
#pragma unroll
    for (int ta = 0; ta < RT; ++ta)
#pragma unroll
      for (int r = 0; r < 4; ++r) {
        const int row = p.row(ta, r);
        io.stJ(1, row, vJm[row] + vs[row] + Rmp.v[ta][r]);
      }
  }
  if constexpr (!RID) {
    __syncthreads();
    if (tid < G::NP) {
      io.stJ(0, tid, vjp[tid] + sm.mv[0][tid]);
      io.stJ(1, tid, vJm[tid] + vs[tid] + sm.mv[1][tid]);
    }
  }
#ifdef VSM_IA_PHASES
  __builtin_amdgcn_s_waitcnt(0);
  VSM_IA_STAMP(11);
  if (threadIdx.x == 0) atomicAdd(&vsm_ia_phase_cycles[15], 1ull);
#endif
}

template <int RT, int KS, bool DSYM>
__global__ __launch_bounds__(ngeo<RT>::NT, ngeo<RT>::WPS) void k_ia_native(int N, int ns, int al16, composite<double> c,
                                                                            added<double> a, int* status) {
  using G = ngeo<RT>;
  extern __shared__ __attribute__((aligned(16))) unsigned char smem_raw[];
  using SM = nsmem<RT, (4 * KS + 2 > 16 * RT)>;
  SM& sm = *reinterpret_cast<SM*>(smem_raw);
  npos<RT> p(sm.P);
  const long long s = blockIdx.x, NN = (long long)N * N;
  const int tid = threadIdx.x;
  nio_ref<RT> io;
  io.N = N;
  io.al16 = al16 != 0;
  io.m[NC_RMP] = c.R_mp + s * NN;
  io.m[NC_RPM] = c.R_pm + s * NN;
  io.m[NC_TPP] = c.T_pp + s * NN;
  io.m[NC_TMM] = c.T_mm + s * NN;
  io.J[0] = c.J0_p + s * N;
  io.J[1] = c.J0_m + s * N;
  io.a[NC_RMP] = a.r_mp + s * a.mat_stride;
  io.a[NC_TPP] = a.t_pp + s * a.mat_stride;
  io.a[NC_RPM] = DSYM ? nullptr : a.r_pm + s * a.mat_stride;
  io.a[NC_TMM] = DSYM ? nullptr : a.t_mm + s * a.mat_stride;
#ifdef VSM_IA_PHASES
  unsigned long long t_ = __builtin_amdgcn_s_memtime();
#endif
  const bool in = tid < N;
  const double j0p = in ? a.j0_p[s * N + tid] : 0.0, j0m = in ? a.j0_m[s * N + tid] : 0.0;
  io.jpre[0] = in ? io.J[0][tid] : 0.0;
  io.jpre[1] = in ? io.J[1][tid] : 0.0;
  nstrip<RT> r_s, t_s;
  io.dma_raw(io.a[NC_RMP], sm.P, p);
  io.dma_raw(io.a[NC_TPP], sm.Q, p);
  io.prefetch(NC_RPM, sm.gjs);
  io.prefetch(NC_TMM, sm.gjs);
  if (tid < G::NP) {
    sm.vec[0][tid] = j0p;
    sm.vec[1][tid] = j0m;
    sm.usg[tid] = (DSYM && (tid % ns) >= 2) ? -1.0 : 1.0;
  }
  __builtin_amdgcn_s_waitcnt(0x0F70);
  __syncthreads();
  io.ld_raw(r_s, sm.P, p);
  io.ld_raw(t_s, sm.Q, p);
  __syncthreads();
  io.dma_raw(io.m[NC_RPM], sm.Q, p);
  io.dma_raw(io.m[NC_TMM], sm.P, p);
#ifdef VSM_IA_PHASES
  __builtin_amdgcn_s_waitcnt(0);
  VSM_IA_STAMP(12);
#endif
  nia_body<RT, KS, DSYM>(sm, p, N, io, r_s, t_s, status);
}

static_assert(sizeof(nsmem<2>) * 8 <= 163840, "two row tiles: eight workgroups per CU");
static_assert(sizeof(nsmem<3>) * 4 <= 163840, "three row tiles: four workgroups per CU");
static_assert(sizeof(nsmem<3, true>) * 3 <= 163840, "three row tiles, mat-vec sources: three workgroups per CU");
static_assert(sizeof(nsmem<4, true>) * 2 <= 163840, "four row tiles: two workgroups per CU");
static_assert(sizeof(nsmem<6, true>) <= 163840 && sizeof(nsmem<6>) <= 163840, "six row tiles: one workgroup per CU");

template <int RT, int KS, bool SRC>
__global__ __launch_bounds__(ngeo<RT>::NT, ngeo<RT>::WPS) void k_layer_native(int n, int gsz, unsigned uvmask, int ndoubl,
                                                                                int toa, const double* __restrict__ pre,
                                                                                nlayer_comps a, int* status) {
  using G = ngeo<RT>;
  extern __shared__ __attribute__((aligned(16))) unsigned char smem_raw[];
  using SM = nsmem<RT, (4 * KS + 2 > 16 * RT)>;
  SM& sm = *reinterpret_cast<SM*>(smem_raw);
  npos<RT> p(sm.P);
  const int s = blockIdx.x, isub = blockIdx.y;
  const double* img = pre + ((long long)isub * gridDim.x + s) * G::PRE_STRIDE;
  double* comp = a.c[isub] + (long long)s * G::COMP_STRIDE;
  nstrip<RT> r_s, t_s;
  ned_body<RT, KS>(sm, p, n, gsz, uvmask, ndoubl, img, r_s, t_s, status);
  if (toa) {
    const ndpar<RT> dp(sm.usg, p);
    if constexpr (!SRC) {
      nst_native(comp + NC_RMP * G::AF, r_s, p);
      nst_native(comp + NC_TPP * G::AF, t_s, p);
    }
    nstrip<RT> d;
    ndsym(d, r_s, dp);
    nst_native(comp + NC_RPM * G::AF, d, p);
    ndsym(d, t_s, dp);
    nst_native(comp + NC_TMM * G::AF, d, p);
    if (threadIdx.x < G::NP) {
      comp[4 * G::AF + threadIdx.x] = sm.vec[0][threadIdx.x];
      comp[4 * G::AF + G::NP + threadIdx.x] = sm.vec[1][threadIdx.x];
    }
    return;
  }
  if constexpr (SRC) nia_body_src<RT, KS>(sm, p, n, comp, r_s, t_s, status);
  else nia_body_native<RT, KS>(sm, p, n, comp, r_s, t_s, status);
}

}

#define VSM_NCAT2(a, b) a##b
#define VSM_NCAT(a, b) VSM_NCAT2(a, b)
#define VSM_NATIVE_DECL(KS) \
  int VSM_NCAT(launch_layer_native_, KS)(int, int, int, unsigned, int, int, int, int, const double*, const nlayer_comps&, int*, \
                                         hipStream_t);                                                                           \
  int VSM_NCAT(launch_ia_native_, KS)(int, int, const composite<double>&, const added<double>&, int*, hipStream_t);

#ifdef VSM_NATIVE_KS
VSM_NATIVE_DECL(VSM_NATIVE_KS)
int VSM_NCAT(launch_layer_native_, VSM_NATIVE_KS)(int S, int nsub, int n, unsigned uvmask, int gsz, int ndoubl, int toa, int src,
                                                  const double* pre, const nlayer_comps& comps, int* status, hipStream_t st) {
  constexpr int KS = VSM_NATIVE_KS;
  constexpr int RT = (KS % 4 == 0 && KS >= 4) ? KS / 4 : (4 * KS + 2 + 15) / 16;
  static_assert(RT >= 1 && RT <= 6, "n <= 96");
  using SM = nsmem<RT, (4 * KS + 2 > 16 * RT)>;
  auto kern = src ? k_layer_native<RT, KS, true> : k_layer_native<RT, KS, false>;
  const int prepared = ensure_dyn_lds(reinterpret_cast<const void*>(kern), sizeof(SM), "hipFuncSetAttribute(k_layer_native)");
  if (prepared) return prepared;
  hipLaunchKernelGGL(kern, dim3(S, nsub), dim3(ngeo<RT>::NT), sizeof(SM), st, n, gsz, uvmask, ndoubl, toa, pre, comps, status);
  VSM_LAUNCH_CHECK("k_layer_native");
  return VSM_OK;
}
#if VSM_NATIVE_KS <= 16
int VSM_NCAT(launch_ia_native_, VSM_NATIVE_KS)(int N, int S, const composite<double>& c, const added<double>& a, int* status,
                                               hipStream_t st) {
  constexpr int KS = VSM_NATIVE_KS;
  constexpr int RT = (KS % 4 == 0 && KS >= 4) ? KS / 4 : (4 * KS + 2 + 15) / 16;
  using SM = nsmem<RT, (4 * KS + 2 > 16 * RT)>;
  auto kd = k_ia_native<RT, KS, true>;
  auto kg = k_ia_native<RT, KS, false>;
  int prepared = ensure_dyn_lds(reinterpret_cast<const void*>(kd), sizeof(SM), "hipFuncSetAttribute(k_ia_native)");
  if (!prepared) prepared = ensure_dyn_lds(reinterpret_cast<const void*>(kg), sizeof(SM), "hipFuncSetAttribute(k_ia_native general)");
  if (prepared) return prepared;
  unsigned long long bits = (unsigned long long)c.R_mp | (unsigned long long)c.R_pm | (unsigned long long)c.T_pp |
                            (unsigned long long)c.T_mm | (unsigned long long)a.r_mp | (unsigned long long)a.t_pp |
                            (unsigned long long)(a.mat_stride * 8);
  if (!a.d_symmetric) bits |= (unsigned long long)a.r_pm | (unsigned long long)a.t_mm;
  const int al16 = ((N & 1) == 0 && (bits & 15ull) == 0) ? 1 : 0;
  if (a.d_symmetric)
    hipLaunchKernelGGL(kd, dim3(S), dim3(ngeo<RT>::NT), sizeof(SM), st, N, a.d_symmetric, al16, c, a, status);
  else
    hipLaunchKernelGGL(kg, dim3(S), dim3(ngeo<RT>::NT), sizeof(SM), st, N, 1, al16, c, a, status);
  VSM_LAUNCH_CHECK("k_ia_native");
  return VSM_OK;
}
#endif
}
#ifdef VSM_IA_PHASES
extern "C" int vsm_debug_ia_phases(unsigned long long* out_h, int reset) {
  if (out_h) (void)hipMemcpyFromSymbol(out_h, HIP_SYMBOL(vsm::vsm_ia_phase_cycles), sizeof(unsigned long long) * 16);
  if (reset) {
    unsigned long long z[16] = {0};
    (void)hipMemcpyToSymbol(HIP_SYMBOL(vsm::vsm_ia_phase_cycles), z, sizeof(z));
  }
  return 0;
}
#endif

#else

VSM_NATIVE_DECL(1)
VSM_NATIVE_DECL(2)
VSM_NATIVE_DECL(3)
VSM_NATIVE_DECL(4)
VSM_NATIVE_DECL(5)
VSM_NATIVE_DECL(6)
VSM_NATIVE_DECL(7)
VSM_NATIVE_DECL(8)
VSM_NATIVE_DECL(9)
VSM_NATIVE_DECL(10)
VSM_NATIVE_DECL(11)
VSM_NATIVE_DECL(12)
VSM_NATIVE_DECL(13)
VSM_NATIVE_DECL(14)
VSM_NATIVE_DECL(15)
VSM_NATIVE_DECL(16)
VSM_NATIVE_DECL(17)
VSM_NATIVE_DECL(18)
VSM_NATIVE_DECL(19)
VSM_NATIVE_DECL(20)
VSM_NATIVE_DECL(21)
VSM_NATIVE_DECL(22)
VSM_NATIVE_DECL(23)
VSM_NATIVE_DECL(24)

namespace {

template <typename ST>
struct nsub_pre {
  int m, gsz;
  int g[4];
  zsrc<ST> z;
};
template <typename ST>
struct npre_args {
  nsub_pre<ST> s[NSUB_MAX];
};
template <int RT, bool MIX, typename ST>
__global__ __launch_bounds__(64 * RT) void k_elemental_native(quad<ST> q, int n, int ndoubl, const ST* __restrict__ dtau,
                                                              const ST* __restrict__ varpi, const ST* __restrict__ tau_sum,
                                                              const ST* __restrict__ F0, npre_args<ST> a,
                                                              double* __restrict__ pre) {
  using G = ngeo<RT>;
  constexpr int NP = G::NP;
  __shared__ double mus[NP], xs[NP], es[NP], ems[NP], wts[NP];
  __shared__ int frow[NP];
  __shared__ int thick_flag;
  const int s = blockIdx.x, isub = blockIdx.y, tid = threadIdx.x;
  const nsub_pre<ST>& sp = a.s[isub];
  const int N = q.N, ns = q.n_stokes, m = sp.m, gsz = sp.gsz;
  const zsrc<ST> z = sp.z;
  const double d = (double)dtau[s], w = (double)varpi[s];
  const int ncomp = MIX ? z.ncomp : 0;
  const long long NNz = (long long)N * N;
  const ST* Zp = z.Zpp + (ncomp ? 0 : (long long)s * z.zs);
  const ST* Zm = z.Zmp + (ncomp ? 0 : (long long)s * z.zs);
  double fk[4] = {0.0, 0.0, 0.0, 0.0};
#pragma unroll
  for (int k = 0; k < 4; ++k)
    if (k < ncomp) fk[k] = (double)z.fcomp[(long long)s * ncomp + k];
  auto zget = [&](const ST* Z, long long zo) {
    if (ncomp == 0) return (double)Z[zo];
    double acc = 0.0;
#pragma unroll
    for (int k = 0; k < 4; ++k)
      if (k < ncomp) acc += fk[k] * (double)Z[k * NNz + zo];
    return acc;
  };
  if (tid < NP) {
    const bool in = tid < n;
    const int ga = sp.g[tid % gsz];
    const int fr = in ? (tid / gsz) * ns + ga : 0;
    const double mu = in ? (double)q.mu[fr] : 1.0;
    const double x = d / mu;
    frow[tid] = fr;
    mus[tid] = mu;
    xs[tid] = x;
    es[tid] = exp(-x);
    ems[tid] = expm1(-x);
    wts[tid] = in ? (double)q.wt[fr] : 0.0;
  }
  if (tid == 0) thick_flag = 0;
  __syncthreads();
  if (tid < n && xs[tid] >= 0.5) thick_flag = 1;
  __syncthreads();
  const bool thick = thick_flag != 0;
  const int i = tid % NP, ph = tid / NP;
  const int ic = min(i, n - 1);
  const double mi = mus[i], xi = xs[i], ai = ems[i], ei = es[i];
  const bool uvi = i < n && sp.g[i % gsz] >= 2;
  const double sg = (ndoubl >= 1 && uvi) ? -1.0 : 1.0;
  double* out = pre + ((long long)isub * gridDim.x + s) * G::PRE_STRIDE;
  double* R = out;
  double* T = out + G::AF;
  const int Kend = ((n + 3) >> 2) << 2;
  const int c1 = Kend, c2 = Kend + 1;
  const bool riders_in = ndoubl > 0 && c2 < NP;
  const int fi = frow[ic];
  for (int j = ph; j < NP; j += 4) {
    if (riders_in && (j == c1 || j == c2)) continue;
    double rv = 0.0, tv = 0.0;
    if (j < n) {
      const double wt = wts[j];
      const double wct = (m == 0) ? wt / 2.0 : wt / 4.0;
      const long long zo = fi + (long long)N * frow[j];
      double rr, tt;
      elemental_pair(w, zget(Zp, zo), zget(Zm, zo), mi, xi, ai, ei, mus[j], xs[j], ems[j], es[j], wct, i == j, thick, rr, tt);
      const bool active = wct > (double)num<ST>::eps();
      if (i < n) {
// ... 128 lines not shown
  if (mm) atomicOr(mask + blockIdx.y, (int)mm);
}

template <typename ST>
struct nguard_args {
  const ST* zp[NSUB_MAX];
  const ST* zm[NSUB_MAX];
  unsigned allowed[NSUB_MAX];
};
template <typename ST>
__global__ __launch_bounds__(256) void k_coupling_guard(int N, int ns, long long mat_stride, nguard_args<ST> a, int* status) {
  const long long NN = (long long)N * N;
  const int im = blockIdx.y;
  const ST* zp = a.zp[im] + mat_stride * blockIdx.x;
  const ST* zm = a.zm[im] + mat_stride * blockIdx.x;
  unsigned mm = 0;
  for (int e = threadIdx.x; e < NN; e += 256) {
    const int i = e % N, j = e / N;
    if (zp[e] != ST(0) || zm[e] != ST(0)) mm |= 1u << (4 * (i % ns) + (j % ns));
  }
  if (mm & ~a.allowed[im]) atomicOr(&status[0], (int)VSM_DEVSTAT_MASK);
}

struct ndiag_args {
  double* comp[NSUB_MAX];
  int gsz[NSUB_MAX];
  int g0[NSUB_MAX];
};
template <typename ST>
__global__ __launch_bounds__(256) void k_native_diag_layer(quad<ST> q, int rt, int n, double scale, int mode, int src,
                                                           const ST* __restrict__ dtau, ndiag_args a) {
  __shared__ double tt[NATIVE_MAX_ROWS];
  const int s = blockIdx.x, isub = blockIdx.y, tid = threadIdx.x;
  const int np = 16 * rt, af = np * np, gsz = a.gsz[isub];
  double* comp = a.comp[isub] + (long long)s * (4 * af + 2 * np);
  if (tid < np) {
    double t = 0.0;
    if (tid < n) {
      const int fr = (tid / gsz) * q.n_stokes + ((a.g0[isub] >> (4 * (tid % gsz))) & 15);
      t = exp(-(double)dtau[s] * scale / (double)q.mu[fr]);
    }
    tt[tid] = t;
    if (mode == 2 && tid < n) {
      const int ix = nnat_idx_rt(rt, tid, tid);
      if (!src) comp[NC_TPP * af + ix] *= t;
      comp[NC_TMM * af + ix] *= t;
    }
  }
  if (mode == 2) return;
  const int toa = mode == 1;
  __syncthreads();
  for (int e = tid; e < af; e += 256) {
    const int half = e & 1, lane = (e >> 1) & 63, unit = (e >> 7) % (2 * rt), w = (e >> 7) / (2 * rt);
    const int i = 16 * (unit >> 1) + (lane >> 4) + 4 * (2 * (unit & 1) + half), j = 16 * w + (lane & 15);
    const double ti = tt[i], tj = tt[j];
    if (toa) {
      const double d = (i == j) ? ti : 0.0;
      if (!src) {
        comp[NC_RMP * af + e] = 0.0;
        comp[NC_TPP * af + e] = d;
      }
      comp[NC_RPM * af + e] = 0.0;
      comp[NC_TMM * af + e] = d;
    } else {
      comp[NC_RPM * af + e] *= ti * tj;
      if (!src) comp[NC_TPP * af + e] *= ti;
      comp[NC_TMM * af + e] *= tj;
    }
  }
  if (tid < np) {
    if (toa) {
      comp[4 * af + tid] = 0.0;
      comp[4 * af + np + tid] = 0.0;
    } else {
      comp[4 * af + tid] *= tt[tid];
    }
  }
}

}

}

namespace vsm {
namespace {

static int stokes_groups(int ns, int coupling, int grp_of[4], int groups[4][4], int gsz[4]) {
  bool adj[4][4] = {};
  for (int a = 0; a < ns; ++a)
    for (int b = 0; b < ns; ++b) {
      const bool on = coupling < 0 || ((coupling >> (4 * a + b)) & 1) || ((coupling >> (4 * b + a)) & 1) || a == b;
      adj[a][b] = on;
    }
  int ng = 0;
  for (int a = 0; a < 4; ++a) grp_of[a] = -1;
  for (int a = 0; a < ns; ++a) {
    if (grp_of[a] >= 0) continue;
    int stack[4], top = 0;
    stack[top++] = a;
    grp_of[a] = ng;
    while (top) {
      const int x = stack[--top];
      for (int b = 0; b < ns; ++b)
        if (adj[x][b] && grp_of[b] < 0) {
          grp_of[b] = ng;
          stack[top++] = b;
        }
    }
    ++ng;
  }
  for (int g = 0; g < ng; ++g) {
    gsz[g] = 0;
    for (int a = 0; a < ns; ++a)
      if (grp_of[a] == g) groups[g][gsz[g]++] = a;
  }
  return ng;
}
static inline int rt_of(int n) {
  const int ks = (n + 3) / 4;
  return (ks % 4 == 0 && ks >= 4) ? ks / 4 : (4 * ks + 2 + 15) / 16;
}
static inline size_t comp_stride_rt(int rt) { return (size_t)4 * (16 * rt) * (16 * rt) + 2 * 16 * rt; }
static inline size_t pre_stride_rt(int rt) { return (size_t)2 * (16 * rt) * (16 * rt) + 3 * 16 * rt; }

static int plan_subs(bool f32, int N, int ns, int nm, const int* m, const int* coupling, std::vector<nat_sub>& subs, size_t S,
                     size_t& total) {
  if (N <= 0 || ns < 1 || ns > 4 || N % ns) {
    set_error("vsm_run: bad N = %d / n_stokes = %d", N, ns);
    return VSM_ERR_INVALID_ARG;
  }
  const int nq = N / ns;
  total = 0;
  subs.clear();
  for (int im = 0; im < nm; ++im) {
    int grp_of[4], groups[4][4], gsz[4];
    const int ng = stokes_groups(ns, coupling ? coupling[im] : -1, grp_of, groups, gsz);
    for (int g = 0; g < ng; ++g) {
      nat_sub sb;
      sb.im = im;
      sb.m = m ? m[im] : 0;
      sb.gsz = gsz[g];
      sb.uvmask = 0;
      for (int k = 0; k < 4; ++k) sb.g[k] = k < gsz[g] ? groups[g][k] : groups[g][0];
      for (int k = 0; k < gsz[g]; ++k)
        if (groups[g][k] >= 2) sb.uvmask |= 1u << k;
      sb.n = nq * gsz[g];
      const int max_rows = f32 ? NATIVE32_MAX_ROWS : NATIVE_MAX_ROWS;
      if (sb.n > max_rows) {
        set_error("vsm_run: a block of %d rows (N = %d, %d coupled Stokes components) is beyond the native kernels (%d)", sb.n, N,
                  gsz[g], max_rows);
        return VSM_ERR_UNSUPPORTED;
      }
      sb.ks = (sb.n + 3) / 4;
      sb.rt = f32 ? native32_rt_of(sb.n) : rt_of(sb.n);
      sb.comp_off = total;
      total += (f32 ? native32_comp_stride(sb.rt) : comp_stride_rt(sb.rt)) * S;
      subs.push_back(sb);
    }
  }
  return VSM_OK;
}

static int launch_layer_native(int ks, int S, int nsub, int n, unsigned uvmask, int gsz, int ndoubl, int toa, int src,
                               const double* pre, const nlayer_comps& comps, int* status, hipStream_t st) {
#define VSM_NL(KS) \
  case KS: return VSM_NCAT(launch_layer_native_, KS)(S, nsub, n, uvmask, gsz, ndoubl, toa, src, pre, comps, status, st);
  switch (ks) {
    VSM_NL(1) VSM_NL(2) VSM_NL(3) VSM_NL(4) VSM_NL(5) VSM_NL(6) VSM_NL(7) VSM_NL(8) VSM_NL(9) VSM_NL(10) VSM_NL(11) VSM_NL(12)
    VSM_NL(13) VSM_NL(14) VSM_NL(15) VSM_NL(16) VSM_NL(17) VSM_NL(18) VSM_NL(19) VSM_NL(20) VSM_NL(21) VSM_NL(22) VSM_NL(23) VSM_NL(24)
    default: break;
  }
#undef VSM_NL
  set_error("launch_layer_native: no kernel for %d k-steps", ks);
  return VSM_ERR_UNSUPPORTED;
}

}
int native_interaction11(int N, int S, const composite<double>& c, const added<double>& a, hipStream_t st) {
  if (N < 1 || N > 64) return VSM_ERR_UNSUPPORTED;
  if (S <= 0) return VSM_OK;
  int* status = device_status();
  if (!status) return VSM_ERR_HIP;
#define VSM_NI(KS) \
  case KS: return VSM_NCAT(launch_ia_native_, KS)(N, S, c, a, status, st);
  switch ((N + 3) / 4) {
    VSM_NI(1) VSM_NI(2) VSM_NI(3) VSM_NI(4) VSM_NI(5) VSM_NI(6) VSM_NI(7) VSM_NI(8) VSM_NI(9) VSM_NI(10) VSM_NI(11) VSM_NI(12)
    VSM_NI(13) VSM_NI(14) VSM_NI(15) VSM_NI(16)
    default: break;
  }
#undef VSM_NI
  return VSM_ERR_UNSUPPORTED;
}
namespace {

template <int RT, typename ST>
static void launch_pre(bool mix, const quad<ST>& q, int S, int nsub, int n, int ndoubl, const ST* dtau, const ST* varpi,
                       const ST* tau_sum, const ST* F0, const npre_args<ST>& a, double* pre, hipStream_t st) {
  const dim3 grid(S, nsub), block(64 * RT);
  if (mix)
    hipLaunchKernelGGL((k_elemental_native<RT, true, ST>), grid, block, 0, st, q, n, ndoubl, dtau, varpi, tau_sum, F0, a, pre);
  else
    hipLaunchKernelGGL((k_elemental_native<RT, false, ST>), grid, block, 0, st, q, n, ndoubl, dtau, varpi, tau_sum, F0, a, pre);
}

static ngroup_map group_map(const vsm_run* run, int im) {
  ngroup_map gm;
  gm.ngroups = 0;
  for (int a = 0; a < 4; ++a) {
    gm.grp_of[a] = gm.pos_in[a] = 0;
    gm.gsz[a] = gm.rt[a] = 1;
    gm.n[a] = 0;
    gm.base[a] = nullptr;
  }
  for (const nat_sub& sb : run->subs) {
    if (sb.im != im) continue;
    const int g = gm.ngroups++;
    gm.gsz[g] = sb.gsz;
    gm.rt[g] = sb.rt;
    gm.n[g] = sb.n;
    gm.base[g] = static_cast<double*>(run->ws) + sb.comp_off;
    for (int k = 0; k < sb.gsz; ++k) {
      gm.grp_of[sb.g[k]] = g;
      gm.pos_in[sb.g[k]] = k;
    }
  }
  return gm;
}

template <typename ST>
static quad<ST> run_quad(const vsm_run* run) {
  return quad<ST>{static_cast<const ST*>(run->mu), static_cast<const ST*>(run->wt), run->N, run->ns, run->i_mu0, (ST)run->mu0};
}

template <typename ST, typename Q>
static int run_create(const Q* q, int S, int nm, const int* m, const int* coupling, void* workspace, size_t workspace_bytes,
                      unsigned flags, vsm_run** run_out) {
  VSM_REQUIRE(q && q->mu && q->wt && run_out && m, "vsm_run_create: null argument");
  VSM_REQUIRE((flags & ~(unsigned)VSM_RUN_SOURCES_ONLY) == 0, "vsm_run_create_ex: unknown flags 0x%x", flags);
  VSM_REQUIRE(S >= 0 && nm >= 1 && nm <= NSUB_MAX, "vsm_run_create: bad S = %d / nm = %d (at most %d moments per run)", S, nm,
              NSUB_MAX);
  vsm_run* run = new vsm_run;
  run->mu = q->mu;
  run->wt = q->wt;
  run->N = q->N;
  run->ns = q->n_stokes;
  run->i_mu0 = q->i_mu0;
  run->mu0 = (double)q->mu0;
  run->elem_size = (int)sizeof(ST);
  run->S = S;
  run->nm = nm;
  run->flags = sizeof(ST) == 8 ? flags : 0u;
  run->m.assign(m, m + nm);
  size_t total = 0;
  const int rc = plan_subs(sizeof(ST) == 4, q->N, q->n_stokes, nm, m, coupling, run->subs, (size_t)S, total);
  if (rc) {
    delete run;
    return rc;
  }
  if (total * sizeof(ST) > workspace_bytes || (total && !workspace) || ((size_t)workspace & 15)) {
    set_error("vsm_run_create: workspace of %zu bytes (16-byte aligned) required, got %zu", total * sizeof(ST), workspace_bytes);
    delete run;
    return VSM_ERR_INVALID_ARG;
  }
  run->ws = workspace;
  run->ws_elems = total;
  run->pure_diag.assign(run->subs.size(), 0);
  for (size_t i = 0; i < run->subs.size(); ++i) {
    const nat_sub& sb = run->subs[i];
    bool placed = false;
    for (auto& cl : run->classes) {
      const nat_sub& h = run->subs[cl[0]];
      if (h.n == sb.n && h.gsz == sb.gsz && h.uvmask == sb.uvmask && (int)cl.size() < NSUB_MAX) {
        cl.push_back((int)i);
        placed = true;
        break;
      }
    }
    if (!placed) run->classes.push_back(std::vector<int>{(int)i});
  }
  *run_out = run;
  return VSM_OK;
}

template <typename ST>
static int run_layer(vsm_run* run, int ndoubl, const ST* dtau, const ST* varpi, const ST* tau_sum, const ST* F0, int ncomp,
                     const ST* const* Zpp, const ST* const* Zmp, long long z_stride, const ST* fcomp, int toa,
                     const int* layer_coupling, void* stream) {
  VSM_REQUIRE(run && dtau && varpi && tau_sum && F0 && Zpp && Zmp, "vsm_run_layer: null argument");
  VSM_REQUIRE(run->elem_size == (int)sizeof(ST), "vsm_run_layer: the run was created for %d-byte arrays", run->elem_size);
  VSM_REQUIRE(ndoubl >= 0 && ndoubl < 60 && ncomp >= 0 && ncomp <= 4 && (ncomp == 0 || fcomp), "vsm_run_layer: bad ndoubl / component mix");
  if (run->S == 0) return VSM_OK;
  hipStream_t st = as_stream(stream);
  int* status = device_status();
  if (!status) return VSM_ERR_HIP;
  const quad<ST> q = run_quad<ST>(run);
  auto trivial = [&](const nat_sub& sb) {
    if (!layer_coupling || layer_coupling[sb.im] < 0) return false;
    for (int a = 0; a < sb.gsz; ++a)
      for (int b = 0; b < sb.gsz; ++b)
        if ((layer_coupling[sb.im] >> (4 * sb.g[a] + sb.g[b])) & 1) return false;
    return true;
  };
  {
    nguard_args<ST> ga;
    for (int k = 0; k < NSUB_MAX; ++k) {
      const int im = k < run->nm ? k : 0;
      VSM_REQUIRE(Zpp[im] && Zmp[im], "vsm_run_layer: null Z of moment %d", im);
      ga.zp[k] = Zpp[im];
      ga.zm[k] = Zmp[im];
      ga.allowed[k] = 0;
    }
    for (const nat_sub& sb : run->subs) {
      if (trivial(sb)) continue;
      for (int a = 0; a < sb.gsz; ++a)
        for (int b = 0; b < sb.gsz; ++b) ga.allowed[sb.im] |= 1u << (4 * sb.g[a] + sb.g[b]);
    }
    const int nmat = ncomp ? ncomp : (z_stride ? run->S : 1);
    hipLaunchKernelGGL((k_coupling_guard<ST>), dim3(nmat, run->nm), dim3(256), 0, st, run->N, run->ns,
                       ncomp ? (long long)run->N * run->N : z_stride, ga, status);
    VSM_LAUNCH_CHECK("k_coupling_guard");
  }
  if constexpr (sizeof(ST) == 4) {
    return native32_run_layer(run, ndoubl, dtau, varpi, tau_sum, F0, ncomp, Zpp, Zmp, z_stride, fcomp, toa, layer_coupling, status, st);
  } else {
  double* const ws = static_cast<double*>(run->ws);
  const int src = (run->flags & VSM_RUN_SOURCES_ONLY) ? 1 : 0;
  size_t pre_total = 0;
  for (const nat_sub& sb : run->subs)
    if (!trivial(sb)) pre_total += pre_stride_rt(sb.rt) * (size_t)run->S;
  double* pre = nullptr;
  if (pre_total) {
    pre = static_cast<double*>(scratch(pre_total * sizeof(double), 3, st));
    if (!pre) return VSM_ERR_HIP;
  }
  size_t off = 0;
  for (const auto& cl : run->classes) {
    const nat_sub& h = run->subs[cl[0]];
    std::vector<int> act, triv[3];
    for (int i : cl) {
      if (!trivial(run->subs[i])) {
        act.push_back(i);
        run->pure_diag[i] = 0;
      } else if (toa) {
        triv[1].push_back(i);
        run->pure_diag[i] = 1;
      } else {
        triv[run->pure_diag[i] ? 2 : 0].push_back(i);
      }
    }
    for (int mode = 0; mode < 3; ++mode) {
      if (triv[mode].empty()) continue;
      ndiag_args da;
      const int nt = (int)triv[mode].size();
      for (int k = 0; k < NSUB_MAX; ++k) {
        const nat_sub& sb = run->subs[triv[mode][k < nt ? k : 0]];
        da.comp[k] = ws + sb.comp_off;
        da.gsz[k] = sb.gsz;
        da.g0[k] = sb.g[0] | (sb.g[1] << 4) | (sb.g[2] << 8) | (sb.g[3] << 12);
      }
      hipLaunchKernelGGL((k_native_diag_layer<ST>), dim3(run->S, nt), dim3(256), 0, st, q, h.rt, h.n, ldexp(1.0, ndoubl), mode, src,
                         dtau, da);
      VSM_LAUNCH_CHECK("k_native_diag_layer");
    }
    const int nsub = (int)act.size();
    if (!nsub) continue;
    npre_args<ST> pa;
    nlayer_comps lc;
    for (int k = 0; k < NSUB_MAX; ++k) {
      const nat_sub& sb = run->subs[act[k < nsub ? k : 0]];
      pa.s[k].m = sb.m;
      pa.s[k].gsz = sb.gsz;
      for (int a = 0; a < 4; ++a) pa.s[k].g[a] = sb.g[a];
      VSM_REQUIRE(Zpp[sb.im] && Zmp[sb.im], "vsm_run_layer: null Z of moment %d", sb.im);
      pa.s[k].z = zsrc<ST>{Zpp[sb.im], Zmp[sb.im], ncomp ? 0 : z_stride, ncomp, fcomp};
      lc.c[k] = ws + sb.comp_off;
    }
    double* pre_cl = pre + off;
    off += pre_stride_rt(h.rt) * (size_t)run->S * nsub;
    switch (h.rt) {
      case 1: launch_pre<1, ST>(ncomp > 0, q, run->S, nsub, h.n, ndoubl, dtau, varpi, tau_sum, F0, pa, pre_cl, st); break;
      case 2: launch_pre<2, ST>(ncomp > 0, q, run->S, nsub, h.n, ndoubl, dtau, varpi, tau_sum, F0, pa, pre_cl, st); break;
      case 3: launch_pre<3, ST>(ncomp > 0, q, run->S, nsub, h.n, ndoubl, dtau, varpi, tau_sum, F0, pa, pre_cl, st); break;
      case 4: launch_pre<4, ST>(ncomp > 0, q, run->S, nsub, h.n, ndoubl, dtau, varpi, tau_sum, F0, pa, pre_cl, st); break;
      case 5: launch_pre<5, ST>(ncomp > 0, q, run->S, nsub, h.n, ndoubl, dtau, varpi, tau_sum, F0, pa, pre_cl, st); break;
      default: launch_pre<6, ST>(ncomp > 0, q, run->S, nsub, h.n, ndoubl, dtau, varpi, tau_sum, F0, pa, pre_cl, st); break;
    }
    VSM_LAUNCH_CHECK("k_elemental_native");
    const int rc = launch_layer_native(h.ks, run->S, nsub, h.n, h.uvmask, h.gsz, ndoubl, toa, src, pre_cl, lc, status, st);
    if (rc) return rc;
  }
  return VSM_OK;
  }
}

template <typename ST, typename CS, bool IMPORT>
static int run_convert(vsm_run* run, const CS* comps, void* stream) {
  VSM_REQUIRE(run && comps, "vsm_run_export / import: null argument");
  VSM_REQUIRE(run->elem_size == (int)sizeof(ST), "vsm_run_export / import: the run was created for %d-byte arrays", run->elem_size);
  if (run->S == 0) return VSM_OK;
  if (IMPORT) run->pure_diag.assign(run->subs.size(), 0);
  for (int im = 0; im < run->nm; ++im) {
    const CS& c = comps[im];
    VSM_REQUIRE(c.R_mp && c.R_pm && c.T_pp && c.T_mm && c.J0_p && c.J0_m, "vsm_run_export / import: null composite array (moment %d)", im);
    const composite<ST> cc{c.R_mp, c.R_pm, c.T_pp, c.T_mm, c.J0_p, c.J0_m};
    if constexpr (sizeof(ST) == 4) {
      const int rc = native32_convert(run, im, cc, IMPORT, as_stream(stream));
      if (rc) return rc;
      continue;
    }
    const ngroup_map gm = group_map(run, im);
    if (IMPORT)
      hipLaunchKernelGGL((k_native_import<ST>), dim3(run->S), dim3(256), 0, as_stream(stream), run->N, run->ns, gm, cc);
    else
      hipLaunchKernelGGL((k_native_export<ST>), dim3(run->S), dim3(256), 0, as_stream(stream), run->N, run->ns,
                         (run->flags & VSM_RUN_SOURCES_ONLY) ? 1 : 0, gm, cc);
    VSM_LAUNCH_CHECK("k_native_export / import");
  }
  return VSM_OK;
}

template <typename ST>
static int stokes_coupling(int N, int n_stokes, int nblocks, const ST* Zpp, const ST* Zmp, int* mask_d, void* stream) {
  VSM_REQUIRE(N > 0 && n_stokes >= 1 && n_stokes <= 4 && N % n_stokes == 0 && nblocks >= 1 && nblocks <= 65535 && Zpp && Zmp &&
                  mask_d, "vsm_stokes_coupling: bad argument");
  hipStream_t st = as_stream(stream);
  VSM_HIP(hipMemsetAsync(mask_d, 0, sizeof(int) * nblocks, st));
  const long long tot = (long long)N * N;
  const int blocks = (int)((tot + 255) / 256 < 16 ? (tot + 255) / 256 : 16);
  hipLaunchKernelGGL((k_stokes_coupling<ST>), dim3(blocks, nblocks), dim3(256), 0, st, N, n_stokes, Zpp, Zmp, mask_d);
  VSM_LAUNCH_CHECK("k_stokes_coupling");
  return VSM_OK;
}

}
}

using namespace vsm;

extern "C" {

static int run_supported(int N, int n_stokes, int coupling, int max_rows) {
  if (N <= 0 || n_stokes < 1 || n_stokes > 4 || N % n_stokes) return 0;
  int grp_of[4], groups[4][4], gsz[4];
  const int ng = stokes_groups(n_stokes, coupling, grp_of, groups, gsz);
  for (int g = 0; g < ng; ++g)
    if ((N / n_stokes) * gsz[g] > max_rows) return 0;
  return 1;
}
int vsm_run_supported(int N, int n_stokes, int coupling) { return run_supported(N, n_stokes, coupling, NATIVE_MAX_ROWS); }
int vsm_run_supported_f32(int N, int n_stokes, int coupling) { return run_supported(N, n_stokes, coupling, NATIVE32_MAX_ROWS); }

size_t vsm_run_workspace_bytes(int N, int n_stokes, int S, int nm, const int* coupling) {
  std::vector<nat_sub> subs;
  size_t total = 0;
  if (S < 0 || nm < 0 || plan_subs(false, N, n_stokes, nm, nullptr, coupling, subs, (size_t)S, total)) return 0;
  return total * sizeof(double);
}
size_t vsm_run_workspace_bytes_f32(int N, int n_stokes, int S, int nm, const int* coupling) {
  std::vector<nat_sub> subs;
  size_t total = 0;
  if (S < 0 || nm < 0 || plan_subs(true, N, n_stokes, nm, nullptr, coupling, subs, (size_t)S, total)) return 0;
  return total * sizeof(float);
}

int vsm_run_create_f64(const vsm_quad_f64* q, int S, int nm, const int* m, const int* coupling, void* workspace,
                       size_t workspace_bytes, vsm_run** run_out) {
  return run_create<double>(q, S, nm, m, coupling, workspace, workspace_bytes, 0u, run_out);
}
int vsm_run_create_f32(const vsm_quad_f32* q, int S, int nm, const int* m, const int* coupling, void* workspace,
                       size_t workspace_bytes, vsm_run** run_out) {
  return run_create<float>(q, S, nm, m, coupling, workspace, workspace_bytes, 0u, run_out);
}
int vsm_run_create_ex_f64(const vsm_quad_f64* q, int S, int nm, const int* m, const int* coupling, void* workspace,
                          size_t workspace_bytes, unsigned flags, vsm_run** run_out) {
  return run_create<double>(q, S, nm, m, coupling, workspace, workspace_bytes, flags, run_out);
}
int vsm_run_create_ex_f32(const vsm_quad_f32* q, int S, int nm, const int* m, const int* coupling, void* workspace,
                          size_t workspace_bytes, unsigned flags, vsm_run** run_out) {
  return run_create<float>(q, S, nm, m, coupling, workspace, workspace_bytes, flags, run_out);
}

int vsm_run_destroy(vsm_run* run) {
  delete run;
  return VSM_OK;
}

int vsm_run_layer_f64(vsm_run* run, int ndoubl, const double* dtau, const double* varpi, const double* tau_sum, const double* F0,
                      int ncomp, const double* const* Zpp, const double* const* Zmp, long long z_stride, const double* fcomp,
                      int toa, const int* layer_coupling, void* stream) {
  return run_layer<double>(run, ndoubl, dtau, varpi, tau_sum, F0, ncomp, Zpp, Zmp, z_stride, fcomp, toa, layer_coupling, stream);
}
int vsm_run_layer_f32(vsm_run* run, int ndoubl, const float* dtau, const float* varpi, const float* tau_sum, const float* F0,
                      int ncomp, const float* const* Zpp, const float* const* Zmp, long long z_stride, const float* fcomp,
                      int toa, const int* layer_coupling, void* stream) {
  return run_layer<float>(run, ndoubl, dtau, varpi, tau_sum, F0, ncomp, Zpp, Zmp, z_stride, fcomp, toa, layer_coupling, stream);
}

int vsm_run_export_f64(vsm_run* run, const vsm_composite_f64* comps, void* stream) {
  return run_convert<double, vsm_composite_f64, false>(run, comps, stream);
}
int vsm_run_export_f32(vsm_run* run, const vsm_composite_f32* comps, void* stream) {
  return run_convert<float, vsm_composite_f32, false>(run, comps, stream);
}
int vsm_run_import_f64(vsm_run* run, const vsm_composite_f64* comps, void* stream) {
  return run_convert<double, vsm_composite_f64, true>(run, comps, stream);
}
int vsm_run_import_f32(vsm_run* run, const vsm_composite_f32* comps, void* stream) {
  return run_convert<float, vsm_composite_f32, true>(run, comps, stream);
}

int vsm_stokes_coupling_f64(int N, int n_stokes, int nblocks, const double* Zpp, const double* Zmp, int* mask_d, void* stream) {
  return stokes_coupling<double>(N, n_stokes, nblocks, Zpp, Zmp, mask_d, stream);
}
int vsm_stokes_coupling_f32(int N, int n_stokes, int nblocks, const float* Zpp, const float* Zmp, int* mask_d, void* stream) {
  return stokes_coupling<float>(N, n_stokes, nblocks, Zpp, Zmp, mask_d, stream);
}

}

#endif
```

vsmartmom.jl_amd/csrc/vsm_native_dev.h:

```cpp
#pragma once
#include "vsm_internal.h"
#include "vsm_lds.h"
#include "vsm_inverse.h"
#include "vsm_elemental.h"

namespace vsm {
namespace {

using nlds_d = __attribute__((address_space(3))) double;
using nlds_i = __attribute__((address_space(3))) int;
__device__ __forceinline__ unsigned nlds_addr(const void* p) {
  return (unsigned)(unsigned long long)(__attribute__((address_space(3))) const void*)p;
}
typedef double nd2_t __attribute__((ext_vector_type(2)));

template <int RT>
struct ngeo {
  static constexpr int NP = 16 * RT;
  static constexpr int NT = 64 * RT;
  static constexpr int AF = NP * NP;
  static constexpr int UNITS = 2 * RT;
  static constexpr int PRE_STRIDE = 2 * AF + 3 * NP;
  static constexpr int COMP_STRIDE = 4 * AF + 2 * NP;
  static constexpr int WPS = RT <= 2 ? 4 : (RT == 3 ? 3 : 2);
};
enum { NC_RMP = 0, NC_RPM = 1, NC_TPP = 2, NC_TMM = 3 };

template <int RT>
__host__ __device__ __forceinline__ int naf_idx(int row, int k) {
  const int ks = k >> 2, kk = k & 3;
  return (ks * RT + (row >> 4)) * 64 + ((kk << 4) | ((row & 15) ^ (kk | ((ks & 3) << 2))));
}
template <int RT>
__host__ __device__ __forceinline__ int nnat_idx(int i, int j) {
  const int w = j >> 4, l15 = j & 15, ta = i >> 4, mm = i & 15, kq = mm & 3, r = mm >> 2;
  const int lane = (kq << 4) | l15, u = 2 * ta + (r >> 1);
  return ((w * 2 * RT + u) * 64 + lane) * 2 + (r & 1);
}

template <int RT>
struct nstrip {
  d4_t v[RT];
  __device__ __forceinline__ void zero() {
#pragma unroll
    for (int a = 0; a < RT; ++a) v[a] = acc_zero<double>();
  }
};

template <int RT>
struct npos {
  int lane, wave, l15, kq, col;
  unsigned fb[4];
  unsigned sb[4];
  __device__ __forceinline__ npos(const void* base) {
    lane = threadIdx.x & 63;
    wave = threadIdx.x >> 6;
    l15 = lane & 15;
    kq = lane >> 4;
    col = 16 * wave + l15;
    const unsigned L = nlds_addr(base);
#pragma unroll
    for (int j = 0; j < 4; ++j) fb[j] = L + 8u * (unsigned)((kq << 4) | (l15 ^ (kq | (j << 2))));
    const int q = l15 >> 2, kk = l15 & 3;
#pragma unroll
    for (int r = 0; r < 4; ++r)
      sb[r] = L + 8u * (unsigned)(((4 * wave + q) * RT * 64) + ((kk << 4) | (kq ^ kk) | ((r ^ q) << 2)));
  }
  __device__ __forceinline__ int row(int ta, int r) const { return 16 * ta + kq + 4 * r; }
  __device__ __forceinline__ const nlds_d* aptr(unsigned dA, int t, int ks) const {
    return reinterpret_cast<const nlds_d*>((unsigned long long)(fb[ks & 3] + dA)) + 64 * (ks * RT + t);
  }
  __device__ __forceinline__ nlds_d* sptr(unsigned dA, int ta, int r) const {
    return reinterpret_cast<nlds_d*>((unsigned long long)(sb[r] + dA)) + 64 * ta;
  }
  __device__ __forceinline__ void opaque() {
#pragma unroll
    for (int j = 0; j < 4; ++j) asm volatile("" : "+v"(fb[j]));
#pragma unroll
    for (int r = 0; r < 4; ++r) asm volatile("" : "+v"(sb[r]));
  }
};

#define VSM_NKSTEP_FENCE() __builtin_amdgcn_sched_barrier(0)

__device__ __forceinline__ double ndpp_swap1(double x) {
  const int lo = __builtin_amdgcn_update_dpp(0, __double2loint(x), 0xB1, 0xf, 0xf, false);
  const int hi = __builtin_amdgcn_update_dpp(0, __double2hiint(x), 0xB1, 0xf, 0xf, false);
  return __hiloint2double(hi, lo);
}

template <int RT, int KS, bool Z = false>
__device__ __forceinline__ void nmm(nstrip<RT>& acc, unsigned dA, const nstrip<RT>& B, npos<RT>& p) {
  p.opaque();
  double a[2][RT];
#pragma unroll
  for (int t = 0; t < RT; ++t) a[0][t] = *p.aptr(dA, t, 0);
#pragma unroll
  for (int ks = 0; ks < KS; ++ks) {
    if (ks + 1 < KS) {
#pragma unroll
      for (int t = 0; t < RT; ++t) a[(ks + 1) & 1][t] = *p.aptr(dA, t, ks + 1);
    }
    const double b = B.v[ks >> 2][ks & 3];
#pragma unroll
    for (int t = 0; t < RT; ++t) acc.v[t] = mfma<double>::mma(a[ks & 1][t], b, (Z && ks == 0) ? acc_zero<double>() : acc.v[t]);
    VSM_NKSTEP_FENCE();
  }
}
template <int RT, int KS>
__device__ __forceinline__ void nmm_c(nstrip<RT>& out, const nstrip<RT>& C0, unsigned dA, const nstrip<RT>& B, npos<RT>& p) {
  p.opaque();
  double a[2][RT];
#pragma unroll
  for (int t = 0; t < RT; ++t) a[0][t] = *p.aptr(dA, t, 0);
#pragma unroll
  for (int ks = 0; ks < KS; ++ks) {
    if (ks + 1 < KS) {
#pragma unroll
      for (int t = 0; t < RT; ++t) a[(ks + 1) & 1][t] = *p.aptr(dA, t, ks + 1);
    }
    const double b = B.v[ks >> 2][ks & 3];
#pragma unroll
    for (int t = 0; t < RT; ++t) out.v[t] = mfma<double>::mma(a[ks & 1][t], b, ks == 0 ? C0.v[t] : out.v[t]);
    VSM_NKSTEP_FENCE();
  }
}
template <int RT, int KS, bool Z1 = false, bool Z2 = false>
__device__ __forceinline__ void nmm2(nstrip<RT>& acc1, nstrip<RT>& acc2, unsigned dA, const nstrip<RT>& B1,
                                     const nstrip<RT>& B2, npos<RT>& p) {
  p.opaque();
  double a[2][RT];
#pragma unroll
  for (int t = 0; t < RT; ++t) a[0][t] = *p.aptr(dA, t, 0);
#pragma unroll
  for (int ks = 0; ks < KS; ++ks) {
    if (ks + 1 < KS) {
#pragma unroll
      for (int t = 0; t < RT; ++t) a[(ks + 1) & 1][t] = *p.aptr(dA, t, ks + 1);
    }
    const double b1 = B1.v[ks >> 2][ks & 3], b2 = B2.v[ks >> 2][ks & 3];
#pragma unroll
    for (int t = 0; t < RT; ++t) {
      acc1.v[t] = mfma<double>::mma(a[ks & 1][t], b1, (Z1 && ks == 0) ? acc_zero<double>() : acc1.v[t]);
      acc2.v[t] = mfma<double>::mma(a[ks & 1][t], b2, (Z2 && ks == 0) ? acc_zero<double>() : acc2.v[t]);
    }
    VSM_NKSTEP_FENCE();
  }
}
template <int RT, int KS, bool Z1 = false, bool Z2 = false>
__device__ __forceinline__ void nmm2a(nstrip<RT>& acc1, unsigned dA1, nstrip<RT>& acc2, unsigned dA2, const nstrip<RT>& B,
                                      npos<RT>& p) {
  p.opaque();
  double a1[2][RT], a2[2][RT];
#pragma unroll
  for (int t = 0; t < RT; ++t) {
    a1[0][t] = *p.aptr(dA1, t, 0);
    a2[0][t] = *p.aptr(dA2, t, 0);
  }
#pragma unroll
  for (int ks = 0; ks < KS; ++ks) {
    if (ks + 1 < KS) {
#pragma unroll
      for (int t = 0; t < RT; ++t) {
        a1[(ks + 1) & 1][t] = *p.aptr(dA1, t, ks + 1);
        a2[(ks + 1) & 1][t] = *p.aptr(dA2, t, ks + 1);
      }
    }
    const double b = B.v[ks >> 2][ks & 3];
#pragma unroll
    for (int t = 0; t < RT; ++t) {
      acc1.v[t] = mfma<double>::mma(a1[ks & 1][t], b, (Z1 && ks == 0) ? acc_zero<double>() : acc1.v[t]);
      acc2.v[t] = mfma<double>::mma(a2[ks & 1][t], b, (Z2 && ks == 0) ? acc_zero<double>() : acc2.v[t]);
    }
    VSM_NKSTEP_FENCE();
  }
}

template <int RT>
__device__ __forceinline__ void nstore(unsigned dA, const nstrip<RT>& s, const npos<RT>& p) {
#pragma unroll
  for (int ta = 0; ta < RT; ++ta)
#pragma unroll
    for (int r = 0; r < 4; ++r) *p.sptr(dA, ta, r) = s.v[ta][r];
}
template <int RT>
__device__ __forceinline__ void nload(nstrip<RT>& s, unsigned dA, const npos<RT>& p) {
#pragma unroll
  for (int ta = 0; ta < RT; ++ta)
#pragma unroll
    for (int r = 0; r < 4; ++r) s.v[ta][r] = *p.sptr(dA, ta, r);
}

template <int RT>
__device__ __forceinline__ void nld_native(nstrip<RT>& s, const double* __restrict__ mat, const npos<RT>& p) {
  const nd2_t* g = reinterpret_cast<const nd2_t*>(mat) + (p.wave * 2 * RT) * 64 + p.lane;
#pragma unroll
  for (int u = 0; u < 2 * RT; ++u) {
    const nd2_t t = g[u * 64];
    s.v[u >> 1][2 * (u & 1)] = t.x;
    s.v[u >> 1][2 * (u & 1) + 1] = t.y;
  }
}
template <int RT>
__device__ __forceinline__ void nst_native(double* __restrict__ mat, const nstrip<RT>& s, const npos<RT>& p) {
  nd2_t* g = reinterpret_cast<nd2_t*>(mat) + (p.wave * 2 * RT) * 64 + p.lane;
#pragma unroll
  for (int u = 0; u < 2 * RT; ++u) {
    nd2_t t;
    t.x = s.v[u >> 1][2 * (u & 1)];
    t.y = s.v[u >> 1][2 * (u & 1) + 1];
    g[u * 64] = t;
  }
}

template <int RT>
__device__ __forceinline__ void ncopy_image(double* L, const double* __restrict__ g, const npos<RT>& p) {
#pragma unroll
  for (int i = 0; i < 2 * RT; ++i) {
    const int blk = (i * RT + p.wave) * 128;
    __builtin_amdgcn_global_load_lds((const __attribute__((address_space(1))) void*)(g + blk + 2 * p.lane),
                                     (__attribute__((address_space(3))) void*)(L + blk), 16, 0, 0);
  }
}

template <int RT>
struct ndpar {
  unsigned rows;
  __device__ __forceinline__ ndpar(const double* usg, const npos<RT>& p) {
    rows = 0;
#pragma unroll
    for (int ta = 0; ta < RT; ++ta)
#pragma unroll
      for (int r = 0; r < 4; ++r) rows |= (usg[p.row(ta, r)] < 0.0 ? 1u : 0u) << (4 * ta + r);
    if (usg[p.col] < 0.0) rows = ~rows;
  }
};
template <int RT>
__device__ __forceinline__ void ndsym(nstrip<RT>& d, const nstrip<RT>& x, const ndpar<RT>& dp) {
  unsigned rows = dp.rows;
  asm volatile("" : "+v"(rows));
#pragma unroll
  for (int ta = 0; ta < RT; ++ta)
#pragma unroll
    for (int r = 0; r < 4; ++r) {
      const int n = 4 * ta + r;
      const unsigned sbit = (rows << (31 - n)) & 0x80000000u;
      d.v[ta][r] = __hiloint2double(__double2hiint(x.v[ta][r]) ^ (int)sbit, __double2loint(x.v[ta][r]));
    }
}

template <int RT, typename SM>
__device__ __forceinline__ double nnorm(const nstrip<RT>& e, int n, SM& sm, int& slot, const npos<RT>& p) {
  double ss = 0;
#pragma unroll
  for (int ta = 0; ta < RT; ++ta)
#pragma unroll
    for (int r = 0; r < 4; ++r) ss = fma(e.v[ta][r], e.v[ta][r], ss);
  ss = (p.col < n) ? ss : 0.0;
  const float ws = wave_sum(to_float_up(ss));
  if (p.lane == 0) sm.red[slot][p.wave] = ws;
  __syncthreads();
  float tot = 0.f;
#pragma unroll
  for (int w = 0; w < RT; ++w) tot += sm.red[slot][w];
  slot ^= 1;
  return (double)(sqrtf(tot) * 1.001f);
}
__device__ __forceinline__ int nseries_order(double nrm) {
  const double tol = num<double>::eps() * 0.25;
  int K = 0;
  if (nrm < 0.3) {
    const double lim = tol * (1.0 - nrm);
    const double n2 = nrm * nrm, n4 = n2 * n2, n8 = n4 * n4, n16 = n8 * n8;
    if (n2 <= lim) K = 1;
    else if (n2 * nrm <= lim) K = 2;
    else if (n4 <= lim) K = 3;
    else if (n4 * nrm <= lim) K = 4;
    else if (n8 <= lim) K = 7;
    else if (n8 * nrm <= lim) K = 8;
    else if (n16 <= lim) K = 15;
    else if (n16 * nrm <= lim) K = 16;
    else if (n16 * n16 <= lim) K = 31;
  }
  return K;
}
template <int RT>
__device__ __forceinline__ void nadd_identity(nstrip<RT>& G, int n, const npos<RT>& p) {
  const bool dl = p.kq == (p.l15 & 3) && p.col < n;
  const int dr = p.l15 >> 2;
#pragma unroll
  for (int ta = 0; ta < RT; ++ta)
    if (ta == p.wave) {
#pragma unroll
      for (int r = 0; r < 4; ++r) G.v[ta][r] += (dl && dr == r) ? 1.0 : 0.0;
    }
}

template <int RT>
__device__ __forceinline__ void ngj_lds(int n, nlds_d* M, nlds_i* piv, nlds_i* src, int* status, const npos<RT>& p) {
  constexpr int NP = 16 * RT;
  constexpr bool TWO = NP > 64;
  const int i0 = p.lane, i1 = p.lane + 64;
  const bool ok0 = i0 < n, ok1 = TWO && i1 < n;
  bool singular = false;
  for (int k = 0; k < n; ++k) {
    const nlds_d* ck = M + k * NP;
    double f0 = ok0 ? ck[i0] : 0.0, f1 = ok1 ? ck[i1] : 0.0;
    const double v0 = (ok0 && i0 >= k) ? fabs(f0) : -1.0, v1 = (ok1 && i1 >= k) ? fabs(f1) : -1.0;
    const double best = wave_max(v0 > v1 ? v0 : v1);
    const unsigned long long m0 = __ballot(v0 >= 0.0 && v0 == best);
    const unsigned long long m1 = __ballot(v1 >= 0.0 && v1 == best);
    const int pr = m0 ? (__ffsll((long long)m0) - 1) : (m1 ? 64 + __ffsll((long long)m1) - 1 : k);
    const double ckk = ck[k], pv = ck[pr];
    const double d = 1.0 / pv;
    singular |= pv == 0.0;
    f0 = (i0 == pr) ? ckk : f0;
    f1 = (i1 == pr) ? ckk : f1;
    if (threadIdx.x == 0) piv[k] = pr;
    __syncthreads();
    for (int j = p.wave; j < n; j += RT) {
      nlds_d* cj = M + j * NP;
      const bool isk = j == k;
      const double a = cj[pr], b = cj[k];
      const double u = isk ? d : a * d;
      double x0 = ok0 ? cj[i0] : 0.0;
      x0 = isk ? 0.0 : ((i0 == pr) ? b : x0);
      x0 = (i0 == k) ? u : fma(-f0, u, x0);
      if (ok0) cj[i0] = x0;
      if constexpr (TWO) {
        double x1 = ok1 ? cj[i1] : 0.0;
        x1 = isk ? 0.0 : ((i1 == pr) ? b : x1);
        x1 = (i1 == k) ? u : fma(-f1, u, x1);
        if (ok1) cj[i1] = x1;
      }
    }
    __syncthreads();
  }
  if (p.wave == 0) {
    if constexpr (TWO) {
      if (p.lane == 0) {
        for (int x = 0; x < n; ++x) src[x] = x;
        for (int k = n - 1; k >= 0; --k) {
          const int q = piv[k];
          if (q != k) {
            const int t = src[k];
            src[k] = src[q];
            src[q] = t;
          }
        }
      }
    } else {
      const int lane = p.lane;
      int s0 = lane;
      const int p0 = (lane < n) ? piv[lane] : lane;
      for (int k = n - 1; k >= 0; --k) {
        const int ku = __builtin_amdgcn_readfirstlane(k);
        const int q = __builtin_amdgcn_readlane(p0, ku);
        if (q != ku) {
          const int sk = __builtin_amdgcn_readlane(s0, ku);
          const int sq = __builtin_amdgcn_readlane(s0, q);
          if (lane == ku) s0 = sq;
          if (lane == q) s0 = sk;
        }
      }
      src[lane] = s0;
    }
    if (p.lane == 0) {
      if (singular) atomicOr(&status[0], (int)VSM_DEVSTAT_SINGULAR);
      atomicAdd(&status[1], 1);
    }
  }
  __syncthreads();
}

struct ninv_ctx {
  unsigned dW;
  double* W;
  int* gjs;
  int* status;
};

template <int RT, int KS>
__device__ __forceinline__ void ninvert_slow_body(int K, nstrip<RT>& E, nstrip<RT>& G, int n, const ninv_ctx& cx, npos<RT>& p);
template <int RT, int KS, bool REGS>
__device__ __attribute__((noinline)) void ninvert_slow(int K, nstrip<RT>& E_in, nstrip<RT>& G_out, int n, const ninv_ctx& cx_in,
                                                       npos<RT>& p_in) {
  if constexpr (REGS) {
    nstrip<RT> E = E_in, G;
    npos<RT> p = p_in;
    const ninv_ctx cx = cx_in;
    ninvert_slow_body<RT, KS>(K, E, G, n, cx, p);
    G_out = G;
  } else {
    ninvert_slow_body<RT, KS>(K, E_in, G_out, n, cx_in, p_in);
  }
}
template <int RT, int KS>
__device__ __forceinline__ void ninvert_slow_body(int K, nstrip<RT>& E, nstrip<RT>& G, int n, const ninv_ctx& cx, npos<RT>& p) {
  constexpr int NP = 16 * RT;
  if (K == 0) {
    if (p.col < n) {
      double* mc = cx.W + p.col * NP + p.kq;
#pragma unroll
      for (int ta = 0; ta < RT; ++ta)
#pragma unroll
        for (int r = 0; r < 4; ++r) mc[16 * ta + 4 * r] = (p.row(ta, r) == p.col ? 1.0 : 0.0) - E.v[ta][r];
    }
    __syncthreads();
    nlds_d* M = reinterpret_cast<nlds_d*>((unsigned long long)nlds_addr(cx.W));
    nlds_i* piv = reinterpret_cast<nlds_i*>((unsigned long long)nlds_addr(cx.gjs));
    constexpr int PV = NP > 64 ? NP : 64;
    ngj_lds<RT>(n, M, piv, piv + PV, cx.status, p);
    const bool cok = p.col < n;
    const nlds_d* gc = M + (cok ? piv[PV + p.col] : 0) * NP + p.kq;
#pragma unroll
    for (int ta = 0; ta < RT; ++ta)
#pragma unroll
      for (int r = 0; r < 4; ++r) {
        const double v = gc[16 * ta + 4 * r];
        G.v[ta][r] = (cok && p.row(ta, r) < n) ? v : 0.0;
      }
    return;
  }
#pragma unroll
  for (int ta = 0; ta < RT; ++ta)
#pragma unroll
    for (int r = 0; r < 4; ++r) E.v[ta][r] = (p.col < n) ? E.v[ta][r] : 0.0;
  G = E;
  nadd_identity(G, n, p);
  nstore(cx.dW, E, p);
  __syncthreads();
  int cur = 1;
  for (int lvl = 0; lvl < 5; ++lvl) {
    nstrip<RT> W2;
    W2.zero();
    nmm<RT, KS>(W2, cx.dW, E, p);
    cur *= 2;
    if (K == cur) {
#pragma unroll
      for (int ta = 0; ta < RT; ++ta) G.v[ta] += W2.v[ta];
      break;
    }
    __syncthreads();
    nstore(cx.dW, W2, p);
    __syncthreads();
    {
      nstrip<RT> T;
      T.zero();
      nmm<RT, KS>(T, cx.dW, G, p);
#pragma unroll
      for (int ta = 0; ta < RT; ++ta) G.v[ta] += T.v[ta];
    }
    if (K == 2 * cur - 1) break;
    E = W2;
  }
}

template <int RT, int KS, bool REGS = false>
__device__ __forceinline__ void ninvert(int K, nstrip<RT>& E, nstrip<RT>& G, int n, const ninv_ctx& cx, npos<RT>& p) {
  if (K < 1 || K > 8) {
    nstrip<RT> Es = E, Gs;
    npos<RT> ps = p;
    ninvert_slow<RT, KS, REGS>(K, Es, Gs, n, cx, ps);
    G = Gs;
    return;
  }
  if (K == 1) {
    G = E;
  } else {
    nstore(cx.dW, E, p);
    __syncthreads();
    nmm_c<RT, KS>(G, E, cx.dW, E, p);
    for (int j = 2; j < K; ++j) {
      nstrip<RT> X;
      nload(X, cx.dW, p);
      nmm<RT, KS>(X, cx.dW, G, p);
      G = X;
    }
  }
  nadd_identity(G, n, p);
}
template <int RT, int KS>
__device__ __forceinline__ void ninvert7(nstrip<RT>& E, nstrip<RT>& G, int n, const ninv_ctx& cx, npos<RT>& p) {
  nstore(cx.dW, E, p);
  __syncthreads();
  nstrip<RT> X, Y;
  nmm_c<RT, KS>(X, E, cx.dW, E, p);
  nload(Y, cx.dW, p);
  nmm<RT, KS>(Y, cx.dW, X, p);
#pragma unroll
  for (int ta = 0; ta < RT; ++ta) X.v[ta] = Y.v[ta] - X.v[ta];
  nmm<RT, KS, true>(G, cx.dW, X, p);
  __syncthreads();
  nstore(cx.dW, G, p);
#pragma unroll
  for (int ta = 0; ta < RT; ++ta) G.v[ta] += Y.v[ta];
  __syncthreads();
  nmm<RT, KS>(G, cx.dW, Y, p);
  nadd_identity(G, n, p);
}
__device__ __forceinline__ int ninv_order(double nrm, int* status) {
  if (!(nrm < 1e300) && threadIdx.x == 0) atomicOr(&status[0], (int)VSM_DEVSTAT_NONFINITE);
  return nseries_order(nrm);
}

template <int RT, bool ON>
struct nmv_slots {};
template <int RT>
struct nmv_slots<RT, true> {
  double mv[2][16 * RT];
};
template <int RT, bool MV = false>
struct nsmem : nmv_slots<RT, MV> {
  double P[ngeo<RT>::AF];
  double Q[ngeo<RT>::AF];
  double vec[8][ngeo<RT>::NP];
  double usg[ngeo<RT>::NP];
  float red[2][8];
  int flags[4];
  int gjs[2 * (ngeo<RT>::NP > 64 ? ngeo<RT>::NP : 64)];
};

template <int RT, int KS>
__device__ __forceinline__ void nmv_rows(unsigned dA, const double* x, double sc, double* out, npos<RT>& p) {
  unsigned ab[4];
#pragma unroll
  for (int j = 0; j < 4; ++j) {
    ab[j] = p.fb[j] + dA + 512u * (unsigned)p.wave;
    asm volatile("" : "+v"(ab[j]));
  }
  unsigned xb = nlds_addr(x) + 8u * (unsigned)p.kq;
  asm volatile("" : "+v"(xb));
  double acc = 0.0;
#pragma unroll
  for (int ks = 0; ks < KS; ++ks) {
    const double a = *(reinterpret_cast<const nlds_d*>((unsigned long long)ab[ks & 3]) + 64 * ks * RT);
    const double xv = *(reinterpret_cast<const nlds_d*>((unsigned long long)xb) + 4 * ks);
    acc = fma(a, xv, acc);
  }
  acc += __shfl_xor(acc, 16);
  acc += __shfl_xor(acc, 32);
  if (p.kq == 0) out[16 * p.wave + p.l15] = acc * sc;
}

}
}
```

vsmartmom.jl_amd/csrc/vsm_native_run.h:

```cpp
#pragma once
#include <vector>

#include "vsm_internal.h"

namespace vsm {

constexpr int NSUB_MAX = VSM_MM_MAX;

struct nat_sub {
  int im;
  int m;
  int gsz, g[4];
  unsigned uvmask;
  int n, rt, ks;
  size_t comp_off;
};

}

struct vsm_run {
  const void *mu, *wt;
  int N, ns, i_mu0;
  double mu0;
  int elem_size;
  int S, nm;
  unsigned flags;
  std::vector<int> m;
  std::vector<vsm::nat_sub> subs;
  std::vector<std::vector<int>> classes;
  void* ws;
  size_t ws_elems;
  std::vector<char> pure_diag;
};

namespace vsm {

constexpr int NATIVE_MAX_ROWS = 96;
constexpr int NATIVE32_MAX_ROWS = 128;
int native32_rt_of(int n);
size_t native32_comp_stride(int rt);
int native32_run_layer(vsm_run* run, int ndoubl, const float* dtau, const float* varpi, const float* tau_sum, const float* F0,
                       int ncomp, const float* const* Zpp, const float* const* Zmp, long long z_stride, const float* fcomp, int toa,
                       const int* layer_coupling, int* status, hipStream_t st);
int native32_convert(vsm_run* run, int im, const composite<float>& c, bool import, hipStream_t st);

}
```

Baseline: 24790.

## Skip zero-weight quadrature tail columns in native layer matrix products

Before any layer step, the run reads the quadrature weights on the host and counts trailing nodes whose weights are all zero. For those tail k-steps the MFMA matrix products, the matrix-vector row products and the series inversion are truncated. Only the diagonal contribution is added back with scalar FMAs, on the reasoning that the weighted columns vanish there apart from the identity part. This adds template instantiations per KS and makes correctness depend on the structure of the zero-weight columns. The mode is turned off on import.

```diff
diff --git a/include/vsmartmom_hip.h b/include/vsmartmom_hip.h
--- a/include/vsmartmom_hip.h
+++ b/include/vsmartmom_hip.h
@@ -348,7 +348,7 @@
                           const float* fcomp, float* Zpp, float* Zmp, void* stream);
 
 typedef struct vsm_run vsm_run;
-enum { VSM_RUN_SOURCES_ONLY = 1 };
+enum { VSM_RUN_SOURCES_ONLY = 1, VSM_RUN_ZW_TAIL = 2 };
 int vsm_run_supported(int N, int n_stokes, int coupling);
 size_t vsm_run_workspace_bytes(int N, int n_stokes, int S, int nm, const int* coupling_h);
 int vsm_run_supported_f32(int N, int n_stokes, int coupling);
@@ -371,6 +371,7 @@
 int vsm_run_export_f32(vsm_run* run, const vsm_composite_f32* comps, void* stream);
 int vsm_run_import_f64(vsm_run* run, const vsm_composite_f64* comps, void* stream);
 int vsm_run_import_f32(vsm_run* run, const vsm_composite_f32* comps, void* stream);
+int vsm_run_zw_tail(vsm_run* run);
 int vsm_run_destroy(vsm_run* run);
 int vsm_stokes_coupling_f64(int N, int n_stokes, int nblocks, const double* Zpp, const double* Zmp, int* mask_d, void* stream);
 int vsm_stokes_coupling_f32(int N, int n_stokes, int nblocks, const float* Zpp, const float* Zmp, int* mask_d, void* stream);
diff --git a/vsmartmom.jl_amd/_lib.py b/vsmartmom.jl_amd/_lib.py
--- a/vsmartmom.jl_amd/_lib.py
+++ b/vsmartmom.jl_amd/_lib.py
@@ -142,6 +142,7 @@
     "vsm_run_layer_{T}": (_I, [_P, _I, _P, _P, _P, _P, _I, _P, _P, _LL, _P, _I, _P, _P]),
     "vsm_run_export_{T}": (_I, [_P, _P, _P]),
     "vsm_run_import_{T}": (_I, [_P, _P, _P]),
+    "vsm_run_zw_tail": (_I, [_P]),
     "vsm_run_destroy": (_I, [_P]),
     "vsm_stokes_coupling_{T}": (_I, [_I, _I, _I, _P, _P, _P, _P]),
     "vsm_level_radiance_work_elems": (_SZ, [_I, _I]),
diff --git a/vsmartmom.jl_amd/core_rt.py b/vsmartmom.jl_amd/core_rt.py
--- a/vsmartmom.jl_amd/core_rt.py
+++ b/vsmartmom.jl_amd/core_rt.py
@@ -21,6 +21,7 @@
 THERMAL_FUSION = True
 NATIVE_RUN = True
 NATIVE_SOURCES_ONLY = True
+NATIVE_ZW_TAIL = True
 NATIVE_DROPIN = True
 REFERENCE_ORDER = False
 
@@ -905,6 +906,8 @@
         flags = 1 if (sources_only and NATIVE_SOURCES_ONLY) else 0
         _lib.call("vsm_run_create_ex", self.dt, C.byref(q), S, nm, marr, carr, _ptr(ws), nbytes, flags, C.byref(run))
         try:
+            if NATIVE_ZW_TAIL and not torch.cuda.is_current_stream_capturing():
+                _lib.check(L.vsm_run_zw_tail(run))
             for iz in range(self.Nz):
                 ly0 = group[0]["layers"][iz]
                 props = [mom["layers"][iz]["props"] for mom in group]
diff --git a/vsmartmom.jl_amd/csrc/vsm_native.hip b/vsmartmom.jl_amd/csrc/vsm_native.hip
--- a/vsmartmom.jl_amd/csrc/vsm_native.hip
+++ b/vsmartmom.jl_amd/csrc/vsm_native.hip
@@ -17,7 +17,7 @@
 
 namespace {
 
-template <int RT, int KS>
+template <int RT, int KS, int KZ = KS>
 __device__ __forceinline__ void ned_body(nsmem<RT, (4 * KS + 2 > 16 * RT)>& sm, npos<RT>& p, int n, int gsz, unsigned uvmask, int ndoubl,
                                          const double* __restrict__ img, nstrip<RT>& r_s, nstrip<RT>& t_s, int* status) {
   using G = ngeo<RT>;
@@ -52,14 +52,14 @@
     nstrip<RT> W, tt;
     const double fW = laneA ? expk : (laneB ? 1.0 : 0.0), fR = laneB ? expk : 1.0;
     if constexpr (!RID) {
-      nmv_rows<RT, KS>(dP, jp, 1.0, sm.mv[0], p);
-      nmv_rows<RT, KS>(dP, jm, expk, sm.mv[1], p);
+      nmv_rows<RT, KS, KZ>(dP, jp, 1.0, sm.mv[0], p);
+      nmv_rows<RT, KS, KZ>(dP, jm, expk, sm.mv[1], p);
     }
     {
       nstrip<RT> Gs;
       {
         nstrip<RT> E;
-        nmm2<RT, KS, true, true>(E, W, dP, r_s, t_s, p);
+        nmm2<RT, KS, true, true, KZ>(E, W, dP, r_s, t_s, p);
         if (own_wave) {
 #pragma unroll
           for (int ta = 0; ta < RT; ++ta)
@@ -76,21 +76,21 @@
             sm.vec[5][tid] = jp[tid] + sm.mv[1][tid];
           }
         }
-        ninvert<RT, KS>(ninv_order(nrm, status), E, Gs, n, cx, p);
-      }
-      nmm<RT, KS, true>(tt, dQ, Gs, p);
+        ninvert<RT, KS, false, KZ>(ninv_order(nrm, status), E, Gs, n, cx, p);
+      }
+      nmm<RT, KS, true, KZ>(tt, dQ, Gs, p);
     }
     nload(t_s, dQ, p);
     __syncthreads();
     nstore(dP, tt, p);
     __syncthreads();
     if constexpr (!RID) {
-      nmv_rows<RT, KS>(dP, sm.vec[4], 1.0, sm.mv[0], p);
-      nmv_rows<RT, KS>(dP, sm.vec[5], 1.0, sm.mv[1], p);
+      nmv_rows<RT, KS, KZ>(dP, sm.vec[4], 1.0, sm.mv[0], p);
+      nmv_rows<RT, KS, KZ>(dP, sm.vec[5], 1.0, sm.mv[1], p);
     }
     {
       nstrip<RT> tn;
-      nmm2<RT, KS, false, true>(r_s, tn, dP, W, t_s, p);
+      nmm2<RT, KS, false, true, KZ>(r_s, tn, dP, W, t_s, p);
       t_s = tn;
     }
     const double expk_step = expk;
@@ -143,7 +143,7 @@
   __syncthreads();
 }
 
-template <int RT, int KS>
+template <int RT, int KS, int KZ = KS>
 __device__ __forceinline__ void nia_body_native(nsmem<RT, (4 * KS + 2 > 16 * RT)>& sm, npos<RT>& p, int n, double* __restrict__ comp, nstrip<RT>& r_s,
                                          nstrip<RT>& t_s, int* status) {
   using G = ngeo<RT>;
@@ -190,12 +190,12 @@
   ndsym(t_s, t_s, dp);
   __syncthreads();
   if constexpr (!RID) {
-    nmv_rows<RT, KS>(dP, vjm, 1.0, sm.mv[0], p);
-    nmv_rows<RT, KS>(dQ, vjm, 1.0, sm.mv[1], p);
+    nmv_rows<RT, KS, KZ>(dP, vjm, 1.0, sm.mv[0], p);
+    nmv_rows<RT, KS, KZ>(dQ, vjm, 1.0, sm.mv[1], p);
   }
   {
     nstrip<RT> E;
-    nmm2<RT, KS, true, true>(E, Z, dP, r_s, t_s, p);
+    nmm2<RT, KS, true, true, KZ>(E, Z, dP, r_s, t_s, p);
     if (own_wave) {
       double* zd = laneB ? vz : sm.vec[7];
 #pragma unroll
@@ -214,12 +214,12 @@
         vs[tid] = sm.mv[1][tid];
       }
     }
-    ninvert<RT, KS>(ninv_order(nrm, status), E, Gs, n, cx, p);
+    ninvert<RT, KS, false, KZ>(ninv_order(nrm, status), E, Gs, n, cx, p);
   }
   nstrip<RT> V;
   {
     nstrip<RT> S;
-    nmm2<RT, KS, true, true>(S, V, dQ, r_s, t_s, p);
+    nmm2<RT, KS, true, true, KZ>(S, V, dQ, r_s, t_s, p);
     if (own_wave) {
       double* sd = laneB ? vs : sm.vec[7];
 #pragma unroll
@@ -236,8 +236,8 @@
   __syncthreads();
   {
     nstrip<RT> X, Y;
-    nmm<RT, KS, true>(X, dP, Gs, p);
-    nmm<RT, KS, true>(Y, dQ, Gs, p);
+    nmm<RT, KS, true, KZ>(X, dP, Gs, p);
+    nmm<RT, KS, true, KZ>(Y, dQ, Gs, p);
     __syncthreads();
     nstore(dP, X, p);
     nstore(dQ, Y, p);
@@ -248,8 +248,8 @@
   if constexpr (PARK) nld_native(Z, R_pm, p); else nld_native(Rmp, R_mp, p);
   __syncthreads();
   if constexpr (!RID) {
-    nmv_rows<RT, KS>(dP, vz, 1.0, sm.mv[0], p);
-    nmv_rows<RT, KS>(dQ, vz, 1.0, sm.mv[1], p);
+    nmv_rows<RT, KS, KZ>(dP, vz, 1.0, sm.mv[0], p);
+    nmv_rows<RT, KS, KZ>(dQ, vz, 1.0, sm.mv[1], p);
   }
   if (own_wave) {
 #pragma unroll
@@ -262,7 +262,7 @@
   }
   {
     nstrip<RT> acc;
-    nmm2<RT, KS, false, true>(r_s, acc, dP, Z, Tpp, p);
+    nmm2<RT, KS, false, true, KZ>(r_s, acc, dP, Z, Tpp, p);
     nst_native(R_pm, r_s, p);
     nst_native(T_pp, acc, p);
     if (laneA) {
@@ -285,7 +285,7 @@
         for (int r = 0; r < 4; ++r) Rmp.v[ta][r] = laneA ? 0.0 : Rmp.v[ta][r];
     }
   }
-  nmm2<RT, KS>(Rmp, V, dQ, Tpp, Z, p);
+  nmm2<RT, KS, false, false, KZ>(Rmp, V, dQ, Tpp, Z, p);
   nst_native(R_mp, Rmp, p);
   nst_native(T_mm, V, p);
   if (laneA) {
@@ -306,7 +306,7 @@
   }
 }
 
-template <int RT, int KS>
+template <int RT, int KS, int KZ = KS>
 __device__ __forceinline__ void nia_body_src(nsmem<RT, (4 * KS + 2 > 16 * RT)>& sm, npos<RT>& p, int n, double* __restrict__ comp,
                                              nstrip<RT>& r_s, nstrip<RT>& t_s, int* status) {
   using G = ngeo<RT>;
@@ -348,14 +348,14 @@
       for (int r = 0; r < 4; ++r) B.v[ta][r] = cin ? B.v[ta][r] : (laneA ? vJp[p.row(ta, r)] : 0.0);
   }
   if constexpr (!RID) {
-    nmv_rows<RT, KS>(dP, vJp, 1.0, sm.mv[0], p);
-    nmv_rows<RT, KS>(dQ, vJp, 1.0, sm.mv[1], p);
+    nmv_rows<RT, KS, KZ>(dP, vJp, 1.0, sm.mv[0], p);
+    nmv_rows<RT, KS, KZ>(dQ, vJp, 1.0, sm.mv[1], p);
   }
   nstrip<RT> E, Bs;
   double nrm;
   {
     nstrip<RT> Pm;
-    nmm2a<RT, KS, true, true>(E, dP, Pm, dQ, B, p);
+    nmm2a<RT, KS, true, true, KZ>(E, dP, Pm, dQ, B, p);
     ndsym(Bs, t_s, dp);
     ndsym(r_s, r_s, dp);
     if (own_wave) {
@@ -382,29 +382,29 @@
   {
     nstrip<RT> Gs;
     const int K = ninv_order(nrm, status);
-    if (K == 7) ninvert7<RT, KS>(E, Gs, n, cx, p);
-    else ninvert<RT, KS>(K, E, Gs, n, cx, p);
+    if (K == 7) ninvert7<RT, KS, KZ>(E, Gs, n, cx, p);
+    else ninvert<RT, KS, false, KZ>(K, E, Gs, n, cx, p);
     __syncthreads();
     nstore(dP, Gs, p);
   }
   __syncthreads();
-  if constexpr (!RID) nmv_rows<RT, KS>(dP, vu, 1.0, vg, p);
+  if constexpr (!RID) nmv_rows<RT, KS, KZ>(dP, vu, 1.0, vg, p);
   {
     nstrip<RT> Tm;
     nld_native(Tm, T_mm, p);
     if constexpr (PARK) nld_native(r_s, R_pm, p);
-    nmm<RT, KS, true>(W, dP, Bs, p);
+    nmm<RT, KS, true, KZ>(W, dP, Bs, p);
     __syncthreads();
     nstore(dP, Tm, p);
   }
   __syncthreads();
   if constexpr (!RID) {
-    nmv_rows<RT, KS>(dP, vg, 1.0, sm.mv[0], p);
-    nmv_rows<RT, KS>(dQ, vg, 1.0, sm.mv[1], p);
+    nmv_rows<RT, KS, KZ>(dP, vg, 1.0, sm.mv[0], p);
+    nmv_rows<RT, KS, KZ>(dQ, vg, 1.0, sm.mv[1], p);
   }
   {
     nstrip<RT> Tn;
-    nmm2a<RT, KS, true, false>(Tn, dP, r_s, dQ, W, p);
+    nmm2a<RT, KS, true, false, KZ>(Tn, dP, r_s, dQ, W, p);
     nst_native(R_pm, r_s, p);
     nst_native(T_mm, Tn, p);
     if (laneA) {
@@ -854,7 +854,7 @@
 static_assert(sizeof(nsmem<4, true>) * 2 <= 163840, "four row tiles: two workgroups per CU");
 static_assert(sizeof(nsmem<6, true>) <= 163840 && sizeof(nsmem<6>) <= 163840, "six row tiles: one workgroup per CU");
 
-template <int RT, int KS, bool SRC>
+template <int RT, int KS, bool SRC, int TZ>
 __global__ __launch_bounds__(ngeo<RT>::NT, ngeo<RT>::WPS) void k_layer_native(int n, int gsz, unsigned uvmask, int ndoubl,
                                                                                 int toa, const double* __restrict__ pre,
                                                                                 nlayer_comps a, int* status) {
@@ -867,7 +867,8 @@
   const double* img = pre + ((long long)isub * gridDim.x + s) * G::PRE_STRIDE;
   double* comp = a.c[isub] + (long long)s * G::COMP_STRIDE;
   nstrip<RT> r_s, t_s;
-  ned_body<RT, KS>(sm, p, n, gsz, uvmask, ndoubl, img, r_s, t_s, status);
+  constexpr int KZ = KS - TZ;
+  ned_body<RT, KS, KZ>(sm, p, n, gsz, uvmask, ndoubl, img, r_s, t_s, status);
   if (toa) {
     const ndpar<RT> dp(sm.usg, p);
     if constexpr (!SRC) {
@@ -885,28 +886,33 @@
     }
     return;
   }
-  if constexpr (SRC) nia_body_src<RT, KS>(sm, p, n, comp, r_s, t_s, status);
-  else nia_body_native<RT, KS>(sm, p, n, comp, r_s, t_s, status);
+  if constexpr (SRC) nia_body_src<RT, KS, KZ>(sm, p, n, comp, r_s, t_s, status);
+  else nia_body_native<RT, KS, KZ>(sm, p, n, comp, r_s, t_s, status);
 }
 
 }
 
 #define VSM_NCAT2(a, b) a##b
 #define VSM_NCAT(a, b) VSM_NCAT2(a, b)
+#define VSM_NATIVE_TZ_MAX 1
 #define VSM_NATIVE_DECL(KS) \
-  int VSM_NCAT(launch_layer_native_, KS)(int, int, int, unsigned, int, int, int, int, const double*, const nlayer_comps&, int*, \
-                                         hipStream_t);                                                                           \
+  int VSM_NCAT(launch_layer_native_, KS)(int, int, int, unsigned, int, int, int, int, int, const double*, const nlayer_comps&, \
+                                         int*, hipStream_t);                                                                     \
   int VSM_NCAT(launch_ia_native_, KS)(int, int, const composite<double>&, const added<double>&, int*, hipStream_t);
 
 #ifdef VSM_NATIVE_KS
 VSM_NATIVE_DECL(VSM_NATIVE_KS)
 int VSM_NCAT(launch_layer_native_, VSM_NATIVE_KS)(int S, int nsub, int n, unsigned uvmask, int gsz, int ndoubl, int toa, int src,
-                                                  const double* pre, const nlayer_comps& comps, int* status, hipStream_t st) {
+                                                  int tz, const double* pre, const nlayer_comps& comps, int* status,
+                                                  hipStream_t st) {
   constexpr int KS = VSM_NATIVE_KS;
   constexpr int RT = (KS % 4 == 0 && KS >= 4) ? KS / 4 : (4 * KS + 2 + 15) / 16;
   static_assert(RT >= 1 && RT <= 6, "n <= 96");
   using SM = nsmem<RT, (4 * KS + 2 > 16 * RT)>;
-  auto kern = src ? k_layer_native<RT, KS, true> : k_layer_native<RT, KS, false>;
+  constexpr int TZ1 = KS - 1 < 1 ? 0 : 1, TZ2 = KS - 1 < VSM_NATIVE_TZ_MAX ? TZ1 : VSM_NATIVE_TZ_MAX;
+  tz = tz < TZ2 ? (tz < TZ1 ? 0 : TZ1) : TZ2;
+  auto kern = src ? (tz == TZ2 ? k_layer_native<RT, KS, true, TZ2> : tz == TZ1 ? k_layer_native<RT, KS, true, TZ1> : k_layer_native<RT, KS, true, 0>)
+                  : (tz == TZ2 ? k_layer_native<RT, KS, false, TZ2> : tz == TZ1 ? k_layer_native<RT, KS, false, TZ1> : k_layer_native<RT, KS, false, 0>);
   const int prepared = ensure_dyn_lds(reinterpret_cast<const void*>(kern), sizeof(SM), "hipFuncSetAttribute(k_layer_native)");
   if (prepared) return prepared;
   hipLaunchKernelGGL(kern, dim3(S, nsub), dim3(ngeo<RT>::NT), sizeof(SM), st, n, gsz, uvmask, ndoubl, toa, pre, comps, status);
@@ -1341,6 +1347,7 @@
         return VSM_ERR_UNSUPPORTED;
       }
       sb.ks = (sb.n + 3) / 4;
+      sb.kz = sb.ks;
       sb.rt = f32 ? native32_rt_of(sb.n) : rt_of(sb.n);
       sb.comp_off = total;
       total += (f32 ? native32_comp_stride(sb.rt) : comp_stride_rt(sb.rt)) * S;
@@ -1350,10 +1357,10 @@
   return VSM_OK;
 }
 
-static int launch_layer_native(int ks, int S, int nsub, int n, unsigned uvmask, int gsz, int ndoubl, int toa, int src,
+static int launch_layer_native(int ks, int tz, int S, int nsub, int n, unsigned uvmask, int gsz, int ndoubl, int toa, int src,
                                const double* pre, const nlayer_comps& comps, int* status, hipStream_t st) {
 #define VSM_NL(KS) \
-  case KS: return VSM_NCAT(launch_layer_native_, KS)(S, nsub, n, uvmask, gsz, ndoubl, toa, src, pre, comps, status, st);
+  case KS: return VSM_NCAT(launch_layer_native_, KS)(S, nsub, n, uvmask, gsz, ndoubl, toa, src, tz, pre, comps, status, st);
   switch (ks) {
     VSM_NL(1) VSM_NL(2) VSM_NL(3) VSM_NL(4) VSM_NL(5) VSM_NL(6) VSM_NL(7) VSM_NL(8) VSM_NL(9) VSM_NL(10) VSM_NL(11) VSM_NL(12)
     VSM_NL(13) VSM_NL(14) VSM_NL(15) VSM_NL(16) VSM_NL(17) VSM_NL(18) VSM_NL(19) VSM_NL(20) VSM_NL(21) VSM_NL(22) VSM_NL(23) VSM_NL(24)
@@ -1421,11 +1428,29 @@
   return quad<ST>{static_cast<const ST*>(run->mu), static_cast<const ST*>(run->wt), run->N, run->ns, run->i_mu0, (ST)run->mu0};
 }
 
+template <typename ST>
+static int zw_tail(vsm_run* run) {
+  const int N = run->N, ns = run->ns, nq = N / ns;
+  std::vector<ST> w((size_t)N);
+  VSM_HIP(hipMemcpy(w.data(), run->wt, sizeof(ST) * (size_t)N, hipMemcpyDefault));
+  int z = 0;
+  for (int node = nq - 1; node >= 0; --node) {
+    bool zero = true;
+    for (int a = 0; a < ns; ++a) zero = zero && w[(size_t)node * ns + a] == ST(0);
+    if (!zero) break;
+    ++z;
+  }
+  if (z == nq) z = 0;
+  for (nat_sub& sb : run->subs) sb.kz = ((nq - z) * sb.gsz + 3) / 4;
+  run->flags |= VSM_RUN_ZW_TAIL;
+  return VSM_OK;
+}
+
 template <typename ST, typename Q>
 static int run_create(const Q* q, int S, int nm, const int* m, const int* coupling, void* workspace, size_t workspace_bytes,
                       unsigned flags, vsm_run** run_out) {
   VSM_REQUIRE(q && q->mu && q->wt && run_out && m, "vsm_run_create: null argument");
-  VSM_REQUIRE((flags & ~(unsigned)VSM_RUN_SOURCES_ONLY) == 0, "vsm_run_create_ex: unknown flags 0x%x", flags);
+  VSM_REQUIRE((flags & ~(unsigned)(VSM_RUN_SOURCES_ONLY | VSM_RUN_ZW_TAIL)) == 0, "vsm_run_create_ex: unknown flags 0x%x", flags);
   VSM_REQUIRE(S >= 0 && nm >= 1 && nm <= NSUB_MAX, "vsm_run_create: bad S = %d / nm = %d (at most %d moments per run)", S, nm,
               NSUB_MAX);
   vsm_run* run = new vsm_run;
@@ -1451,6 +1476,13 @@
     delete run;
     return VSM_ERR_INVALID_ARG;
   }
+  if (run->flags & VSM_RUN_ZW_TAIL) {
+    const int rc2 = zw_tail<ST>(run);
+    if (rc2) {
+      delete run;
+      return rc2;
+    }
+  }
   run->ws = workspace;
   run->ws_elems = total;
   run->pure_diag.assign(run->subs.size(), 0);
@@ -1478,6 +1510,7 @@
   VSM_REQUIRE(run && dtau && varpi && tau_sum && F0 && Zpp && Zmp, "vsm_run_layer: null argument");
   VSM_REQUIRE(run->elem_size == (int)sizeof(ST), "vsm_run_layer: the run was created for %d-byte arrays", run->elem_size);
   VSM_REQUIRE(ndoubl >= 0 && ndoubl < 60 && ncomp >= 0 && ncomp <= 4 && (ncomp == 0 || fcomp), "vsm_run_layer: bad ndoubl / component mix");
+  ++run->layers;
   if (run->S == 0) return VSM_OK;
   hipStream_t st = as_stream(stream);
   int* status = device_status();
@@ -1575,7 +1608,7 @@
       default: launch_pre<6, ST>(ncomp > 0, q, run->S, nsub, h.n, ndoubl, dtau, varpi, tau_sum, F0, pa, pre_cl, st); break;
     }
     VSM_LAUNCH_CHECK("k_elemental_native");
-    const int rc = launch_layer_native(h.ks, run->S, nsub, h.n, h.uvmask, h.gsz, ndoubl, toa, src, pre_cl, lc, status, st);
+    const int rc = launch_layer_native(h.ks, h.ks - h.kz, run->S, nsub, h.n, h.uvmask, h.gsz, ndoubl, toa, src, pre_cl, lc, status, st);
     if (rc) return rc;
   }
   return VSM_OK;
@@ -1587,7 +1620,11 @@
   VSM_REQUIRE(run && comps, "vsm_run_export / import: null argument");
   VSM_REQUIRE(run->elem_size == (int)sizeof(ST), "vsm_run_export / import: the run was created for %d-byte arrays", run->elem_size);
   if (run->S == 0) return VSM_OK;
-  if (IMPORT) run->pure_diag.assign(run->subs.size(), 0);
+  if (IMPORT) {
+    run->pure_diag.assign(run->subs.size(), 0);
+    run->flags &= ~(unsigned)VSM_RUN_ZW_TAIL;
+    for (nat_sub& sb : run->subs) sb.kz = sb.ks;
+  }
   for (int im = 0; im < run->nm; ++im) {
     const CS& c = comps[im];
     VSM_REQUIRE(c.R_mp && c.R_pm && c.T_pp && c.T_mm && c.J0_p && c.J0_m, "vsm_run_export / import: null composite array (moment %d)", im);
@@ -1669,6 +1706,12 @@
   return run_create<float>(q, S, nm, m, coupling, workspace, workspace_bytes, flags, run_out);
 }
 
+int vsm_run_zw_tail(vsm_run* run) {
+  VSM_REQUIRE(run, "vsm_run_zw_tail: null argument");
+  VSM_REQUIRE(run->layers == 0, "vsm_run_zw_tail: the run has taken layer steps already");
+  return run->elem_size == 8 ? zw_tail<double>(run) : VSM_OK;
+}
+
 int vsm_run_destroy(vsm_run* run) {
   delete run;
   return VSM_OK;
diff --git a/vsmartmom.jl_amd/csrc/vsm_native_dev.h b/vsmartmom.jl_amd/csrc/vsm_native_dev.h
--- a/vsmartmom.jl_amd/csrc/vsm_native_dev.h
+++ b/vsmartmom.jl_amd/csrc/vsm_native_dev.h
@@ -89,15 +89,28 @@
   return __hiloint2double(hi, lo);
 }
 
-template <int RT, int KS, bool Z = false>
+template <int RT>
+__device__ __forceinline__ double ndiag(unsigned dA, int ks, const npos<RT>& p) {
+  unsigned b = p.fb[0] - 8u * (unsigned)(p.l15 ^ p.kq);
+  asm volatile("" : "+v"(b));
+  b += dA;
+  return *(reinterpret_cast<const nlds_d*>((unsigned long long)b) + 64 * (ks * RT + (ks >> 2)));
+}
+template <int RT, int KS, int KZ>
+__device__ __forceinline__ void nzw_fix(nstrip<RT>& acc, unsigned dA, const nstrip<RT>& B, const npos<RT>& p) {
+  static_assert(KZ >= 1 && KZ <= KS, "zero-weight tail: 1 <= KZ <= KS");
+#pragma unroll
+  for (int ks = KZ; ks < KS; ++ks) acc.v[ks >> 2][ks & 3] = fma(ndiag<RT>(dA, ks, p), B.v[ks >> 2][ks & 3], acc.v[ks >> 2][ks & 3]);
+}
+template <int RT, int KS, bool Z = false, int KZ = KS>
 __device__ __forceinline__ void nmm(nstrip<RT>& acc, unsigned dA, const nstrip<RT>& B, npos<RT>& p) {
   p.opaque();
   double a[2][RT];
 #pragma unroll
   for (int t = 0; t < RT; ++t) a[0][t] = *p.aptr(dA, t, 0);
 #pragma unroll
-  for (int ks = 0; ks < KS; ++ks) {
-    if (ks + 1 < KS) {
+  for (int ks = 0; ks < KZ; ++ks) {
+    if (ks + 1 < KZ) {
 #pragma unroll
       for (int t = 0; t < RT; ++t) a[(ks + 1) & 1][t] = *p.aptr(dA, t, ks + 1);
     }
@@ -106,16 +119,17 @@
     for (int t = 0; t < RT; ++t) acc.v[t] = mfma<double>::mma(a[ks & 1][t], b, (Z && ks == 0) ? acc_zero<double>() : acc.v[t]);
     VSM_NKSTEP_FENCE();
   }
-}
-template <int RT, int KS>
+  nzw_fix<RT, KS, KZ>(acc, dA, B, p);
+}
+template <int RT, int KS, int KZ = KS>
 __device__ __forceinline__ void nmm_c(nstrip<RT>& out, const nstrip<RT>& C0, unsigned dA, const nstrip<RT>& B, npos<RT>& p) {
   p.opaque();
   double a[2][RT];
 #pragma unroll
   for (int t = 0; t < RT; ++t) a[0][t] = *p.aptr(dA, t, 0);
 #pragma unroll
-  for (int ks = 0; ks < KS; ++ks) {
-    if (ks + 1 < KS) {
+  for (int ks = 0; ks < KZ; ++ks) {
+    if (ks + 1 < KZ) {
 #pragma unroll
       for (int t = 0; t < RT; ++t) a[(ks + 1) & 1][t] = *p.aptr(dA, t, ks + 1);
     }
@@ -124,8 +138,9 @@
     for (int t = 0; t < RT; ++t) out.v[t] = mfma<double>::mma(a[ks & 1][t], b, ks == 0 ? C0.v[t] : out.v[t]);
     VSM_NKSTEP_FENCE();
   }
-}
-template <int RT, int KS, bool Z1 = false, bool Z2 = false>
+  nzw_fix<RT, KS, KZ>(out, dA, B, p);
+}
+template <int RT, int KS, bool Z1 = false, bool Z2 = false, int KZ = KS>
 __device__ __forceinline__ void nmm2(nstrip<RT>& acc1, nstrip<RT>& acc2, unsigned dA, const nstrip<RT>& B1,
                                      const nstrip<RT>& B2, npos<RT>& p) {
   p.opaque();
@@ -133,8 +148,8 @@
 #pragma unroll
   for (int t = 0; t < RT; ++t) a[0][t] = *p.aptr(dA, t, 0);
 #pragma unroll
-  for (int ks = 0; ks < KS; ++ks) {
-    if (ks + 1 < KS) {
+  for (int ks = 0; ks < KZ; ++ks) {
+    if (ks + 1 < KZ) {
 #pragma unroll
       for (int t = 0; t < RT; ++t) a[(ks + 1) & 1][t] = *p.aptr(dA, t, ks + 1);
     }
@@ -146,8 +161,14 @@
     }
     VSM_NKSTEP_FENCE();
   }
-}
-template <int RT, int KS, bool Z1 = false, bool Z2 = false>
+#pragma unroll
+  for (int ks = KZ; ks < KS; ++ks) {
+    const double d = ndiag<RT>(dA, ks, p);
+    acc1.v[ks >> 2][ks & 3] = fma(d, B1.v[ks >> 2][ks & 3], acc1.v[ks >> 2][ks & 3]);
+    acc2.v[ks >> 2][ks & 3] = fma(d, B2.v[ks >> 2][ks & 3], acc2.v[ks >> 2][ks & 3]);
+  }
+}
+template <int RT, int KS, bool Z1 = false, bool Z2 = false, int KZ = KS>
 __device__ __forceinline__ void nmm2a(nstrip<RT>& acc1, unsigned dA1, nstrip<RT>& acc2, unsigned dA2, const nstrip<RT>& B,
                                       npos<RT>& p) {
   p.opaque();
@@ -158,8 +179,8 @@
     a2[0][t] = *p.aptr(dA2, t, 0);
   }
 #pragma unroll
-  for (int ks = 0; ks < KS; ++ks) {
-    if (ks + 1 < KS) {
+  for (int ks = 0; ks < KZ; ++ks) {
+    if (ks + 1 < KZ) {
 #pragma unroll
       for (int t = 0; t < RT; ++t) {
         a1[(ks + 1) & 1][t] = *p.aptr(dA1, t, ks + 1);
@@ -174,6 +195,8 @@
     }
     VSM_NKSTEP_FENCE();
   }
+  nzw_fix<RT, KS, KZ>(acc1, dA1, B, p);
+  nzw_fix<RT, KS, KZ>(acc2, dA2, B, p);
 }
 
 template <int RT>
@@ -456,7 +479,7 @@
   }
 }
 
-template <int RT, int KS, bool REGS = false>
+template <int RT, int KS, bool REGS = false, int KZ = KS>
 __device__ __forceinline__ void ninvert(int K, nstrip<RT>& E, nstrip<RT>& G, int n, const ninv_ctx& cx, npos<RT>& p) {
   if (K < 1 || K > 8) {
     nstrip<RT> Es = E, Gs;
@@ -470,33 +493,33 @@
   } else {
     nstore(cx.dW, E, p);
     __syncthreads();
-    nmm_c<RT, KS>(G, E, cx.dW, E, p);
+    nmm_c<RT, KS, KZ>(G, E, cx.dW, E, p);
     for (int j = 2; j < K; ++j) {
       nstrip<RT> X;
       nload(X, cx.dW, p);
-      nmm<RT, KS>(X, cx.dW, G, p);
+      nmm<RT, KS, false, KZ>(X, cx.dW, G, p);
       G = X;
     }
   }
   nadd_identity(G, n, p);
 }
-template <int RT, int KS>
+template <int RT, int KS, int KZ = KS>
 __device__ __forceinline__ void ninvert7(nstrip<RT>& E, nstrip<RT>& G, int n, const ninv_ctx& cx, npos<RT>& p) {
   nstore(cx.dW, E, p);
   __syncthreads();
   nstrip<RT> X, Y;
-  nmm_c<RT, KS>(X, E, cx.dW, E, p);
+  nmm_c<RT, KS, KZ>(X, E, cx.dW, E, p);
   nload(Y, cx.dW, p);
-  nmm<RT, KS>(Y, cx.dW, X, p);
+  nmm<RT, KS, false, KZ>(Y, cx.dW, X, p);
 #pragma unroll
   for (int ta = 0; ta < RT; ++ta) X.v[ta] = Y.v[ta] - X.v[ta];
-  nmm<RT, KS, true>(G, cx.dW, X, p);
+  nmm<RT, KS, true, KZ>(G, cx.dW, X, p);
   __syncthreads();
   nstore(cx.dW, G, p);
 #pragma unroll
   for (int ta = 0; ta < RT; ++ta) G.v[ta] += Y.v[ta];
   __syncthreads();
-  nmm<RT, KS>(G, cx.dW, Y, p);
+  nmm<RT, KS, false, KZ>(G, cx.dW, Y, p);
   nadd_identity(G, n, p);
 }
 __device__ __forceinline__ int ninv_order(double nrm, int* status) {
@@ -521,7 +544,7 @@
   int gjs[2 * (ngeo<RT>::NP > 64 ? ngeo<RT>::NP : 64)];
 };
 
-template <int RT, int KS>
+template <int RT, int KS, int KZ = KS>
 __device__ __forceinline__ void nmv_rows(unsigned dA, const double* x, double sc, double* out, npos<RT>& p) {
   unsigned ab[4];
 #pragma unroll
@@ -533,11 +556,20 @@
   asm volatile("" : "+v"(xb));
   double acc = 0.0;
 #pragma unroll
-  for (int ks = 0; ks < KS; ++ks) {
+  for (int ks = 0; ks < KZ; ++ks) {
     const double a = *(reinterpret_cast<const nlds_d*>((unsigned long long)ab[ks & 3]) + 64 * ks * RT);
     const double xv = *(reinterpret_cast<const nlds_d*>((unsigned long long)xb) + 4 * ks);
     acc = fma(a, xv, acc);
   }
+  if constexpr (KZ < KS) {
+    const int row = 16 * p.wave + p.l15;
+    if (row >= 4 * KZ && row < 4 * KS && p.kq == (row & 3)) {
+      const nlds_d* Ad = reinterpret_cast<const nlds_d*>((unsigned long long)(p.fb[0] - 8u * (unsigned)(p.l15 ^ p.kq) - 128u * (unsigned)p.kq + dA));
+      const double d = Ad[naf_idx<RT>(row, row)];
+      const double xv = *(reinterpret_cast<const nlds_d*>((unsigned long long)nlds_addr(x)) + row);
+      acc = fma(d, xv, acc);
+    }
+  }
   acc += __shfl_xor(acc, 16);
   acc += __shfl_xor(acc, 32);
   if (p.kq == 0) out[16 * p.wave + p.l15] = acc * sc;
diff --git a/vsmartmom.jl_amd/csrc/vsm_native_run.h b/vsmartmom.jl_amd/csrc/vsm_native_run.h
--- a/vsmartmom.jl_amd/csrc/vsm_native_run.h
+++ b/vsmartmom.jl_amd/csrc/vsm_native_run.h
@@ -13,6 +13,7 @@
   int gsz, g[4];
   unsigned uvmask;
   int n, rt, ks;
+  int kz;
   size_t comp_off;
 };
 
@@ -30,6 +31,7 @@
   std::vector<std::vector<int>> classes;
   void* ws;
   size_t ws_elems;
+  int layers = 0;
   std::vector<char> pure_diag;
 };
 
```

Result: faster. 26180 (median of 6 runs) (+5.6%).
